# YyzHarry/imbalanced-regression

Hardware: NVIDIA H100
Metric: images/sec (higher is better)
Workload: dtype bf16

## Files before the change

imbalanced-regression_b200/_convlib.py:

```python
from ctypes import c_float, c_int, c_int64, c_size_t, c_void_p

import _lib

P = c_void_p
_I9 = [c_int] * 9

_lib.register({
    "dirb200_conv_prep_weights": (c_int, [P, c_int, c_int, c_int, c_int, c_int, P, P, P]),
    "dirb200_input_to_s2d": (c_int, [P, c_int, c_int, c_int, P, P]),
    "dirb200_conv_fprop": (c_int, [P, P, P] + _I9 + [c_int, P]),
    "dirb200_conv_dgrad": (c_int, [P, P, P] + _I9 + [P]),
    "dirb200_conv_wgrad_workspace_bytes": (c_size_t, _I9 + [c_int]),
    "dirb200_conv_wgrad": (c_int, [P, P, P, P, c_size_t] + _I9 + [c_int, c_int, P]),
    "dirb200_conv_plan": (c_int, _I9 + [c_int, c_int, P]),
    "dirb200_bn_eval_coeffs": (c_int, [c_int, P, P, c_float, P, P, P, P, P]),
    "dirb200_conv_fprop_bn_stats": (c_int, [P, P, P] + _I9 + [c_int, P, P, P]),
    "dirb200_conv_fprop_affine": (c_int, [P, P, P] + _I9 + [P, P, P, c_int, P]),
    "dirb200_conv_dgrad_bn_moments": (c_int, [P, P, P] + _I9 + [P, P, P, P, P, P]),
    "dirb200_bn_finalize_layout": (c_int, [P, P, c_int64, c_int, P, P, c_float, c_float, P, P, P, P, P, P, P]),
    "dirb200_bn_bwd_coeffs_layout": (c_int, [P, P, c_int64, c_int, P, P, P, P, P, P, P]),
})
```

imbalanced-regression_b200/csrc/conv.cuh:

```cuda
#pragma once
#include "common.cuh"

namespace dirb200 {

struct ConvShape {
  int n, h, w, cin, cout, kh, kw, stride, pad, ho, wo;
};

struct StatLayout {
  int rows, n_tiles, bn, group;
};

int conv_fprop(const __nv_bfloat16* x, const __nv_bfloat16* w, __nv_bfloat16* y, const ConvShape& s, bool stem,
               cudaStream_t st, float* stat_partial = nullptr, StatLayout* layout = nullptr);
struct ConvEpilogue {
  const float* scale;
  const float* shift;
  const __nv_bfloat16* residual;
  bool relu;
};
int conv_fprop_affine(const __nv_bfloat16* x, const __nv_bfloat16* w, __nv_bfloat16* out, const ConvShape& s,
                      const ConvEpilogue& epi, cudaStream_t st);
struct DgradBnMoments {
  const __nv_bfloat16* y;
  const float *scale, *shift;
  float* partial;
  StatLayout* layout;
};
bool conv_dgrad_fuses_bn_moments(const ConvShape& s);
int conv_dgrad(const __nv_bfloat16* dy, const __nv_bfloat16* wt, __nv_bfloat16* dx, const ConvShape& s,
               cudaStream_t st, const DgradBnMoments* bnm = nullptr);
int conv_wgrad_splits(const ConvShape& s);
size_t conv_wgrad_workspace_bytes(const ConvShape& s);
int conv_wgrad_partials(const __nv_bfloat16* x, const __nv_bfloat16* dy, float* partial, const ConvShape& s, bool stem,
                        int* splits_out, cudaStream_t st);
int wgrad_reduce(const float* workspace, int splits, float* dw, const ConvShape& s, bool stem, bool accumulate,
                 cudaStream_t st);
int conv_wgrad(const __nv_bfloat16* x, const __nv_bfloat16* dy, float* dw, float* workspace, const ConvShape& s,
               bool stem, bool accumulate, cudaStream_t st);
struct WgradReduceDesc {
  const float* partial;
  size_t w_off;
  int splits, cout, cin, kh, kw, stem;
};
int wgrad_reduce_all(const WgradReduceDesc* descs_dev, int nlayers, float* grads, cudaStream_t st);
struct PrepDesc {
  size_t w_off;
  int cout, cin, kh, kw, stem;
  __nv_bfloat16 *wf, *wd;
  FastDiv fd_cin, fd_cout, fd_taps;
};
inline PrepDesc make_prep_desc(size_t w_off, int cout, int cin, int kh, int kw, int stem, __nv_bfloat16* wf,
                               __nv_bfloat16* wd) {
  PrepDesc d{w_off, cout, cin, kh, kw, stem, wf, wd, {}, {}, {}};
  d.fd_cin = make_fastdiv((uint32_t)cin);
  d.fd_cout = make_fastdiv((uint32_t)cout);
  d.fd_taps = make_fastdiv((uint32_t)(kh * kw));
  return d;
}
int conv_plan(const ConvShape& s, bool stem, int op, int* plan);
int prep_weights_all(const float* params, const PrepDesc* descs_dev, int nlayers, cudaStream_t st);
int prep_weights(const float* w, int cout, int cin, int kh, int kw, bool stem, __nv_bfloat16* wf, __nv_bfloat16* wd,
                 cudaStream_t st);
int input_to_s2d(const float* x, int n, int h, int w, __nv_bfloat16* out, cudaStream_t st);

}
```

imbalanced-regression_b200/csrc/conv_api.cu:

```cuda
#include "common.cuh"
#include "conv.cuh"

namespace dirb200 {

__global__ void prep_weights_kernel(const float* __restrict__ w, int cout, int cin, int kh, int kw,
                                    __nv_bfloat16* __restrict__ wf, __nv_bfloat16* __restrict__ wd) {
  const int64_t total = (int64_t)cout * cin * kh * kw;
  for (int64_t i = blockIdx.x * (int64_t)blockDim.x + threadIdx.x; i < total; i += (int64_t)gridDim.x * blockDim.x) {
    int c = (int)(i % cin);
    int64_t t = i / cin;
    int s = (int)(t % kw); t /= kw;
    int r = (int)(t % kh);
    int co = (int)(t / kh);
    const float v = w[(((int64_t)co * cin + c) * kh + r) * kw + s];
    const __nv_bfloat16 b = __float2bfloat16_rn(v);
    wf[i] = b;
    if (wd) wd[(((int64_t)c * kh + r) * kw + s) * cout + co] = b;
  }
}

__global__ void prep_stem_weights_kernel(const float* __restrict__ w, int cout, __nv_bfloat16* __restrict__ wf) {
  const int total = cout * 256;
  for (int i = blockIdx.x * blockDim.x + threadIdx.x; i < total; i += gridDim.x * blockDim.x) {
    const int co = i >> 8, k = i & 255;
    const int rp = k >> 6, sp = (k >> 4) & 3, ph = (k >> 3) & 1, pw = (k >> 2) & 1, c = k & 3;
    const int r = 2 * rp + ph - 1, s = 2 * sp + pw - 1;
    float v = 0.f;
    if (c < 3 && r >= 0 && s >= 0 && r < 7 && s < 7) v = w[((co * 3 + c) * 7 + r) * 7 + s];
    wf[i] = __float2bfloat16_rn(v);
  }
}

__global__ void input_to_s2d_kernel(const float* __restrict__ x, int n, int h, int w, __nv_bfloat16* __restrict__ out) {
  const int h2 = h / 2, w2 = w / 2;
  const int64_t total = (int64_t)n * h2 * w2;
  for (int64_t i = blockIdx.x * (int64_t)blockDim.x + threadIdx.x; i < total; i += (int64_t)gridDim.x * blockDim.x) {
    const int xw = (int)(i % w2);
    const int yh = (int)((i / w2) % h2);
    const int b = (int)(i / ((int64_t)w2 * h2));
    __align__(16) __nv_bfloat16 v[16];
#pragma unroll
    for (int ph = 0; ph < 2; ++ph)
#pragma unroll
      for (int pw = 0; pw < 2; ++pw) {
#pragma unroll
        for (int c = 0; c < 3; ++c)
          v[(ph * 2 + pw) * 4 + c] =
              __float2bfloat16_rn(x[(((int64_t)b * 3 + c) * h + (2 * yh + ph)) * w + (2 * xw + pw)]);
        v[(ph * 2 + pw) * 4 + 3] = __float2bfloat16_rn(0.f);
      }
    uint4* o = reinterpret_cast<uint4*>(out + i * 16);
    o[0] = reinterpret_cast<uint4*>(v)[0];
    o[1] = reinterpret_cast<uint4*>(v)[1];
  }
}

__global__ void wgrad_reduce_kernel(const float* __restrict__ partial, int splits, int cout, int cin, int kh, int kw,
                                    int accumulate, float* __restrict__ dw) {
  const int64_t ktot = (int64_t)kh * kw * cin;
  const int64_t total = ktot * cout;
  const int64_t i = blockIdx.x * (int64_t)blockDim.x + threadIdx.x;
  if (i >= total) return;
  const int co = (int)(i / ktot);
  const int64_t k = i - (int64_t)co * ktot;
  float acc = 0.f;
  for (int sp = 0; sp < splits; ++sp) acc += partial[(int64_t)sp * total + i];
  const int c = (int)(k % cin);
  const int t = (int)(k / cin);
  float* o = dw + ((int64_t)co * cin + c) * (kh * kw) + t;
  *o = accumulate ? *o + acc : acc;
}

__global__ void wgrad_reduce_stem_kernel(const float* __restrict__ partial, int splits, int cout, int accumulate,
                                         float* __restrict__ dw) {
  const int total = 256 * cout;
  for (int i = blockIdx.x * blockDim.x + threadIdx.x; i < total; i += gridDim.x * blockDim.x) {
    const int co = i >> 8, k = i & 255;
    const int rp = k >> 6, sp_ = (k >> 4) & 3, ph = (k >> 3) & 1, pw = (k >> 2) & 1, c = k & 3;
    const int r = 2 * rp + ph - 1, s = 2 * sp_ + pw - 1;
    if (c >= 3 || r < 0 || s < 0) continue;
    float acc = 0.f;
    for (int sp = 0; sp < splits; ++sp) acc += partial[(int64_t)sp * total + i];
    float* o = dw + ((co * 3 + c) * 7 + r) * 7 + s;
    *o = accumulate ? *o + acc : acc;
  }
}

__global__ void __launch_bounds__(256)
wgrad_reduce_all_kernel(const WgradReduceDesc* __restrict__ descs, float* __restrict__ grads) {
  const WgradReduceDesc d = descs[blockIdx.y];
  float* dw = grads + d.w_off;
  if (d.stem) {
    const int total = 256 * d.cout;
    for (int i = blockIdx.x * blockDim.x + threadIdx.x; i < total; i += gridDim.x * blockDim.x) {
      const int co = i >> 8, k = i & 255;
      const int rp = k >> 6, sp_ = (k >> 4) & 3, ph = (k >> 3) & 1, pw = (k >> 2) & 1, c = k & 3;
      const int r = 2 * rp + ph - 1, s = 2 * sp_ + pw - 1;
      if (c >= 3 || r < 0 || s < 0) continue;
      float acc = 0.f;
      for (int sp = 0; sp < d.splits; ++sp) acc += d.partial[(int64_t)sp * total + i];
      dw[((co * 3 + c) * 7 + r) * 7 + s] += acc;
    }
    return;
  }
  const int64_t ktot = (int64_t)d.kh * d.kw * d.cin;
  const int64_t total = ktot * d.cout;
  const int taps = d.kh * d.kw;
  for (int64_t i = blockIdx.x * (int64_t)blockDim.x + threadIdx.x; i < total; i += (int64_t)gridDim.x * blockDim.x) {
    const float* p = d.partial + i;
    float a0 = 0.f, a1 = 0.f, a2 = 0.f, a3 = 0.f;
    int sp = 0;
    for (; sp + 4 <= d.splits; sp += 4) {
      a0 += p[(int64_t)sp * total];
      a1 += p[(int64_t)(sp + 1) * total];
      a2 += p[(int64_t)(sp + 2) * total];
      a3 += p[(int64_t)(sp + 3) * total];
    }
    for (; sp < d.splits; ++sp) a0 += p[(int64_t)sp * total];
    const int64_t co = i / ktot, k = i - co * ktot;
    const int c = (int)(k % d.cin), t = (int)(k / d.cin);
    dw[(co * d.cin + c) * taps + t] += (a0 + a1) + (a2 + a3);
  }
}

int wgrad_reduce_all(const WgradReduceDesc* descs_dev, int nlayers, float* grads, cudaStream_t st) {
  if (nlayers <= 0) return DIRB200_OK;
  wgrad_reduce_all_kernel<<<dim3(2 * num_sms(), nlayers), 256, 0, st>>>(descs_dev, grads);
  DIRB_LAUNCHED();
  return DIRB200_OK;
}

__global__ void prep_weights_all_kernel(const float* __restrict__ params, const PrepDesc* __restrict__ descs) {
  const PrepDesc d = descs[blockIdx.y];
  const float* w = params + d.w_off;
  if (d.stem) {
    const int total = d.cout * 256;
    for (int i = blockIdx.x * blockDim.x + threadIdx.x; i < total; i += gridDim.x * blockDim.x) {
      const int co = i >> 8, k = i & 255;
      const int rp = k >> 6, sp = (k >> 4) & 3, ph = (k >> 3) & 1, pw = (k >> 2) & 1, c = k & 3;
      const int r = 2 * rp + ph - 1, s = 2 * sp + pw - 1;
      float v = 0.f;
      if (c < 3 && r >= 0 && s >= 0 && r < 7 && s < 7) v = w[((co * 3 + c) * 7 + r) * 7 + s];
      d.wf[i] = __float2bfloat16_rn(v);
    }
    return;
  }
  const uint32_t taps = (uint32_t)(d.kh * d.kw);
  const uint32_t total = (uint32_t)d.cout * (uint32_t)d.cin * taps;
  const uint32_t stride = gridDim.x * blockDim.x;
  for (uint32_t i = blockIdx.x * blockDim.x + threadIdx.x; i < total; i += stride) {
    uint32_t t, c, co, tap;
    d.fd_cin.divmod(i, t, c);
    d.fd_taps.divmod(t, co, tap);
    d.wf[i] = __float2bfloat16_rn(w[((size_t)co * d.cin + c) * taps + tap]);
  }
  if (!d.wd) return;
  for (uint32_t i = blockIdx.x * blockDim.x + threadIdx.x; i < total; i += stride) {
    uint32_t t, c, co, tap;
    d.fd_cout.divmod(i, t, co);
    d.fd_taps.divmod(t, c, tap);
    d.wd[i] = __float2bfloat16_rn(w[((size_t)co * d.cin + c) * taps + tap]);
  }
}

int prep_weights_all(const float* params, const PrepDesc* descs_dev, int nlayers, cudaStream_t st) {
  prep_weights_all_kernel<<<dim3(96, nlayers), 256, 0, st>>>(params, descs_dev);
  DIRB_LAUNCHED();
  return DIRB200_OK;
}

static inline int grid1d(int64_t n, int block = 256) {
  int64_t g = (n + block - 1) / block;
  const int64_t cap = 8 * (int64_t)num_sms();
  return (int)(g < 1 ? 1 : (g > cap ? cap : g));
}

int prep_weights(const float* w, int cout, int cin, int kh, int kw, bool stem, __nv_bfloat16* wf, __nv_bfloat16* wd,
                 cudaStream_t st) {
  if (stem) {
    prep_stem_weights_kernel<<<grid1d((int64_t)cout * 256), 256, 0, st>>>(w, cout, wf);
  } else {
    prep_weights_kernel<<<grid1d((int64_t)cout * cin * kh * kw), 256, 0, st>>>(w, cout, cin, kh, kw, wf, wd);
  }
  DIRB_LAUNCHED();
  return DIRB200_OK;
}

int input_to_s2d(const float* x, int n, int h, int w, __nv_bfloat16* out, cudaStream_t st) {
  input_to_s2d_kernel<<<grid1d((int64_t)n * (h / 2) * (w / 2)), 256, 0, st>>>(x, n, h, w, out);
  DIRB_LAUNCHED();
  return DIRB200_OK;
}

int wgrad_reduce(const float* workspace, int splits, float* dw, const ConvShape& s, bool stem, bool accumulate,
                 cudaStream_t st) {
  if (stem)
    wgrad_reduce_stem_kernel<<<grid1d(256 * (int64_t)s.cout), 256, 0, st>>>(workspace, splits, s.cout, accumulate, dw);
  else
  {
    const int64_t total = (int64_t)s.kh * s.kw * s.cin * s.cout;
    wgrad_reduce_kernel<<<(unsigned)((total + 255) / 256), 256, 0, st>>>(workspace, splits, s.cout, s.cin, s.kh, s.kw,
                                                                         accumulate, dw);
  }
  DIRB_LAUNCHED();
  return DIRB200_OK;
}

int conv_wgrad(const __nv_bfloat16* x, const __nv_bfloat16* dy, float* dw, float* workspace, const ConvShape& s,
               bool stem, bool accumulate, cudaStream_t st) {
  int splits = 1;
  if (int rc = conv_wgrad_partials(x, dy, workspace, s, stem, &splits, st)) return rc;
  return wgrad_reduce(workspace, splits, dw, s, stem, accumulate, st);
}

static int to_shape(int n, int h, int w, int cin, int cout, int kh, int kw, int stride, int pad, int stem,
                    ConvShape* s) {
  if (stem) {
    DIRB_CHECK_ARG(cin == 3 && kh == 7 && kw == 7 && stride == 2 && pad == 3 && h % 2 == 0 && w % 2 == 0,
                   "stem conv must be 3->Cout 7x7 stride 2 pad 3 on even H, W");
    *s = ConvShape{n, h / 2, w / 2, 16, cout, 4, 4, 1, 2, h / 2, w / 2};
  } else {
    DIRB_CHECK_ARG(n > 0 && h > 0 && w > 0 && kh > 0 && kw > 0 && stride > 0 && pad >= 0, "bad conv shape");
    *s = ConvShape{n, h, w, cin, cout, kh, kw, stride, pad, (h + 2 * pad - kh) / stride + 1,
                   (w + 2 * pad - kw) / stride + 1};
  }
  return DIRB200_OK;
}

static int conv_job_shape_ok(const char* who, int k, int cout, int cin, int kh, int kw, int stem) {
  DIRB_CHECK_ARG(cout > 0 && cin > 0 && kh > 0 && kw > 0, "%s: job %d has a non-positive size (%d, %d, %d, %d)", who, k,
                 cout, cin, kh, kw);
  DIRB_CHECK_ARG(!stem || (cin == 3 && kh == 7 && kw == 7), "%s: job %d: the stem must be 3x7x7", who, k);
  const int64_t weights = (int64_t)cout * cin * kh * kw;
  DIRB_CHECK_ARG(weights < (int64_t(1) << 31) && (!stem || 256 * (int64_t)cout < (int64_t(1) << 31)),
                 "%s: job %d has 2^31 or more weights", who, k);
  return DIRB200_OK;
}

}

using namespace dirb200;

extern "C" {

int dirb200_conv_prep_weights(const float* w, int cout, int cin, int kh, int kw, int stem, void* w_fprop,
                              void* w_dgrad, void* stream) {
  DIRB_CHECK_ARG(w && w_fprop && cout > 0 && cin > 0, "conv_prep_weights: bad arguments");
  DIRB_CHECK_ARG(!stem || (cin == 3 && kh == 7 && kw == 7), "conv_prep_weights: stem must be 3x7x7");
  return prep_weights(w, cout, cin, kh, kw, stem != 0, (__nv_bfloat16*)w_fprop, (__nv_bfloat16*)w_dgrad,
                      as_stream(stream));
}

int dirb200_input_to_s2d(const float* x_nchw, int n, int h, int w, void* out_bf16, void* stream) {
  DIRB_CHECK_ARG(x_nchw && out_bf16 && n > 0 && h > 0 && w > 0 && h % 2 == 0 && w % 2 == 0,
                 "input_to_s2d: bad arguments");
  return input_to_s2d(x_nchw, n, h, w, (__nv_bfloat16*)out_bf16, as_stream(stream));
}

int dirb200_conv_fprop(const void* x, const void* w_fprop, void* y, int n, int h, int w, int cin, int cout, int kh,
                       int kw, int stride, int pad, int stem, void* stream) {
  DIRB_CHECK_ARG(x && w_fprop && y, "conv_fprop: null pointer");
  ConvShape s;
  if (int rc = to_shape(n, h, w, cin, cout, kh, kw, stride, pad, stem, &s)) return rc;
  return conv_fprop((const __nv_bfloat16*)x, (const __nv_bfloat16*)w_fprop, (__nv_bfloat16*)y, s, stem != 0,
                    as_stream(stream));
}

int dirb200_conv_dgrad(const void* dy, const void* w_dgrad, void* dx, int n, int h, int w, int cin, int cout, int kh,
                       int kw, int stride, int pad, void* stream) {
  DIRB_CHECK_ARG(dy && w_dgrad && dx, "conv_dgrad: null pointer");
  ConvShape s;
  if (int rc = to_shape(n, h, w, cin, cout, kh, kw, stride, pad, 0, &s)) return rc;
  return conv_dgrad((const __nv_bfloat16*)dy, (const __nv_bfloat16*)w_dgrad, (__nv_bfloat16*)dx, s,
                    as_stream(stream));
}

size_t dirb200_conv_wgrad_workspace_bytes(int n, int h, int w, int cin, int cout, int kh, int kw, int stride, int pad,
                                          int stem) {
  ConvShape s;
  if (to_shape(n, h, w, cin, cout, kh, kw, stride, pad, stem, &s)) return 0;
  return conv_wgrad_workspace_bytes(s);
}

int dirb200_conv_wgrad(const void* x, const void* dy, float* dw, void* workspace, size_t workspace_bytes, int n, int h,
                       int w, int cin, int cout, int kh, int kw, int stride, int pad, int stem, int accumulate,
                       void* stream) {
  DIRB_CHECK_ARG(x && dy && dw && workspace, "conv_wgrad: null pointer");
  ConvShape s;
  if (int rc = to_shape(n, h, w, cin, cout, kh, kw, stride, pad, stem, &s)) return rc;
  if (workspace_bytes < conv_wgrad_workspace_bytes(s)) {
    set_error("conv_wgrad: workspace too small (%zu < %zu)", workspace_bytes, conv_wgrad_workspace_bytes(s));
    return DIRB200_ERR_WORKSPACE;
  }
  return conv_wgrad((const __nv_bfloat16*)x, (const __nv_bfloat16*)dy, dw, (float*)workspace, s, stem != 0,
                    accumulate != 0, as_stream(stream));
}

static void layout_to_host(const StatLayout& l, int* layout_host) {
  layout_host[0] = l.rows; layout_host[1] = l.n_tiles; layout_host[2] = l.bn; layout_host[3] = l.group;
}

int dirb200_conv_fprop_bn_stats(const void* x, const void* w_fprop, void* y, int n, int h, int w, int cin, int cout,
                                int kh, int kw, int stride, int pad, int stem, float* partial, int* layout_host,
                                void* stream) {
  DIRB_CHECK_ARG(x && w_fprop && y && partial && layout_host, "conv_fprop_bn_stats: null pointer");
  ConvShape s;
  if (int rc = to_shape(n, h, w, cin, cout, kh, kw, stride, pad, stem, &s)) return rc;
  StatLayout lay{};
  if (int rc = conv_fprop((const __nv_bfloat16*)x, (const __nv_bfloat16*)w_fprop, (__nv_bfloat16*)y, s, stem != 0,
                          as_stream(stream), partial, &lay))
    return rc;
  layout_to_host(lay, layout_host);
  return DIRB200_OK;
}

int dirb200_conv_fprop_affine(const void* x, const void* w_fprop, void* out, int n, int h, int w, int cin, int cout,
                              int kh, int kw, int stride, int pad, const float* scale, const float* shift,
                              const void* residual, int relu, void* stream) {
  DIRB_CHECK_ARG(x && w_fprop && out, "conv_fprop_affine: null pointer");
  ConvShape s;
  if (int rc = to_shape(n, h, w, cin, cout, kh, kw, stride, pad, 0, &s)) return rc;
  return conv_fprop_affine((const __nv_bfloat16*)x, (const __nv_bfloat16*)w_fprop, (__nv_bfloat16*)out, s,
                           ConvEpilogue{scale, shift, (const __nv_bfloat16*)residual, relu != 0}, as_stream(stream));
}

int dirb200_conv_dgrad_bn_moments(const void* dy, const void* w_dgrad, void* dx, int n, int h, int w, int cin, int cout,
                                  int kh, int kw, int stride, int pad, const void* y_prev, const float* scale,
                                  const float* shift, float* partial, int* layout_host, void* stream) {
  DIRB_CHECK_ARG(dy && w_dgrad && dx && y_prev && scale && shift && partial && layout_host,
                 "conv_dgrad_bn_moments: null pointer");
  ConvShape s;
  if (int rc = to_shape(n, h, w, cin, cout, kh, kw, stride, pad, 0, &s)) return rc;
  StatLayout lay{};
  const DgradBnMoments bm{(const __nv_bfloat16*)y_prev, scale, shift, partial, &lay};
  if (int rc = conv_dgrad((const __nv_bfloat16*)dy, (const __nv_bfloat16*)w_dgrad, (__nv_bfloat16*)dx, s,
                          as_stream(stream), &bm))
    return rc;
  layout_to_host(lay, layout_host);
  return DIRB200_OK;
}

int dirb200_conv_plan(int n, int h, int w, int cin, int cout, int kh, int kw, int stride, int pad, int stem, int op,
                      int* plan7) {
  DIRB_CHECK_ARG(plan7 && op >= 0 && op <= 2, "conv_plan: bad arguments");
  ConvShape s;
  if (int rc = to_shape(n, h, w, cin, cout, kh, kw, stride, pad, stem, &s)) return rc;
  return conv_plan(s, stem != 0, op, plan7);
}

int dirb200_prep_weights_all(const float* params, const dirb200_prep_job* jobs_host, int njobs, void* stream) {
  DIRB_CHECK_ARG(params && jobs_host, "prep_weights_all: null pointer");
  DIRB_CHECK_ARG(njobs >= 1 && njobs <= 65535, "prep_weights_all: njobs must be 1 .. 65535 (got %d)", njobs);
  std::vector<PrepDesc> descs;
  for (int k = 0; k < njobs; ++k) {
    const dirb200_prep_job& j = jobs_host[k];
    DIRB_CHECK_ARG(j.w_fprop, "prep_weights_all: job %d has a null w_fprop", k);
    DIRB_CHECK_ARG(j.w_off >= 0, "prep_weights_all: job %d has a negative w_off", k);
    if (int rc = conv_job_shape_ok("prep_weights_all", k, j.cout, j.cin, j.kh, j.kw, j.stem)) return rc;
    DIRB_CHECK_ARG(!j.stem || !j.w_dgrad, "prep_weights_all: job %d: the stem has no dgrad operand (w_dgrad must be null)",
                   k);
    descs.push_back(make_prep_desc((size_t)j.w_off, j.cout, j.cin, j.kh, j.kw, j.stem ? 1 : 0,
                                   (__nv_bfloat16*)j.w_fprop, (__nv_bfloat16*)j.w_dgrad));
  }
  cudaStream_t st = as_stream(stream);
  return with_device_table(descs, st, [&](const PrepDesc* d) { return prep_weights_all(params, d, njobs, st); });
}

int dirb200_wgrad_reduce_all(const dirb200_wgrad_reduce_job* jobs_host, int njobs, float* grads, void* stream) {
  DIRB_CHECK_ARG(jobs_host && grads, "wgrad_reduce_all: null pointer");
  DIRB_CHECK_ARG(njobs >= 1 && njobs <= 65535, "wgrad_reduce_all: njobs must be 1 .. 65535 (got %d)", njobs);
  std::vector<WgradReduceDesc> descs;
  for (int k = 0; k < njobs; ++k) {
    const dirb200_wgrad_reduce_job& j = jobs_host[k];
    DIRB_CHECK_ARG(j.partial, "wgrad_reduce_all: job %d has a null partial", k);
    DIRB_CHECK_ARG(j.w_off >= 0, "wgrad_reduce_all: job %d has a negative w_off", k);
    DIRB_CHECK_ARG(j.splits >= 1, "wgrad_reduce_all: job %d: splits must be at least 1 (got %d)", k, j.splits);
    if (int rc = conv_job_shape_ok("wgrad_reduce_all", k, j.cout, j.cin, j.kh, j.kw, j.stem)) return rc;
    descs.push_back(WgradReduceDesc{j.partial, (size_t)j.w_off, j.splits, j.cout, j.cin, j.kh, j.kw, j.stem ? 1 : 0});
  }
  cudaStream_t st = as_stream(stream);
  return with_device_table(descs, st, [&](const WgradReduceDesc* d) { return wgrad_reduce_all(d, njobs, grads, st); });
}

}
```

imbalanced-regression_b200/csrc/conv_igemm.cu:

```cuda
#include <stdlib.h>
#include "common.cuh"
#include "tc.cuh"
#include "conv.cuh"

namespace dirb200 {
using namespace tc;

constexpr int BM = 128;
constexpr int BK = 64;
constexpr int kProducerThreads = 128;
constexpr int kThreads = 384;
constexpr int kMaxTaps = 25;
constexpr int kMaxSmemBytes = 232448;

struct IgemmParams {
  const __nv_bfloat16* src;
  int n, hs, ws, cs;
  int hm, wm;
  int kh, kw, stride, pad;
  int transposed;
  int cls_on, cls_py, cls_px, full_h, full_w;
  int ntaps_c;
  int tap_list[kMaxTaps];
  long long tap_eoff[kMaxTaps];
  unsigned short tap_r[kMaxTaps], tap_s[kMaxTaps];
  FastDiv fd_hw, fd_wm, fd_cpb, fd_kw, fd_ntiles, fd_persplit;
  int cpb;
  long long pixels;
  int num_kblocks;
  int kblocks_per_split;
  int total_chunks;
  int m_tiles, n_tiles;
  int num_tiles;
  int a_mode;
  int i2c_stride, i2c_lo;
  int ldc;
  void* out;
  float* stat_out;
  const float* epi_scale;
  const float* epi_shift;
  const __nv_bfloat16* epi_res;
  int epi_relu;
  const __nv_bfloat16* bst_y;
  const float* bst_scale;
  const float* bst_shift;
};

template <int BN, bool STAGED_EPI>
struct Cfg {
  static constexpr int kABytes = BM * BK * 2;
  static constexpr int kBBytes = BN * BK * 2;
  static constexpr int kStageBytes = kABytes + kBBytes;
  static constexpr int kStages = BN == 128 ? (STAGED_EPI ? 5 : 6) : 8;
  static constexpr int kBarOffset = kStages * kStageBytes;
  static constexpr int kStageRowBytes = BN * 2 + 16;
  static constexpr int kEpiWarpBytes = 16 * kStageRowBytes;
  static constexpr int kEpiOffset = kBarOffset + 256;
  static constexpr int kStatWarpBytes = 2 * BN * 4;
  static constexpr int kStatOffset = kEpiOffset + (STAGED_EPI ? 8 * kEpiWarpBytes : 0);
  static constexpr int kSmemBytes = kStatOffset + (STAGED_EPI ? 8 * kStatWarpBytes : 0) + 1024;
  static_assert(kSmemBytes <= kMaxSmemBytes, "shared memory budget");
};

__device__ __forceinline__ uint32_t pack_pixel(long long p, const IgemmParams& P) {
  if (p >= P.pixels) return 0u;
  uint32_t n, rem, y, x;
  P.fd_hw.divmod(static_cast<uint32_t>(p), n, rem);
  P.fd_wm.divmod(rem, y, x);
  return 0x80000000u | (n << 18) | (y << 9) | x;
}

struct RowPre {
  int nb, yb, xb;
};
__device__ __forceinline__ RowPre row_pre(const IgemmParams& P, uint32_t pk) {
  RowPre rp;
  const int n = (pk >> 18) & 0x1FFF;
  int y = (pk >> 9) & 0x1FF, x = pk & 0x1FF;
  if (P.cls_on) {
    y = 2 * y + P.cls_py;
    x = 2 * x + P.cls_px;
  }
  rp.nb = n * P.hs;
  if (!P.transposed) {
    rp.yb = y * P.stride - P.pad;
    rp.xb = x * P.stride - P.pad;
  } else {
    rp.yb = y + P.pad;
    rp.xb = x + P.pad;
  }
  if (!(pk >> 31)) rp.yb = -(1 << 28);
  return rp;
}

__device__ __forceinline__ const __nv_bfloat16* tap_source(const IgemmParams& P, const RowPre& rp, int r, int s,
                                                           int coff, bool& ok) {
  int hi, wi;
  ok = true;
  if (!P.transposed) {
    hi = rp.yb + r;
    wi = rp.xb + s;
  } else {
    hi = rp.yb - r;
    wi = rp.xb - s;
    if (P.stride == 2) {
      ok = ((hi | wi) & 1) == 0;
      hi >>= 1;
      wi >>= 1;
    }
  }
  ok = ok && static_cast<unsigned>(hi) < static_cast<unsigned>(P.hs) &&
       static_cast<unsigned>(wi) < static_cast<unsigned>(P.ws);
  return ok ? P.src + (static_cast<size_t>(rp.nb + hi) * P.ws + wi) * P.cs + coff : P.src;
}

template <int BN, bool WGRAD, bool STEM, bool ATMA = false, bool AFFINE = false, bool BSTAT = false>
__global__ void __launch_bounds__(kThreads, 1)
igemm_kernel(const __grid_constant__ CUtensorMap tmap_b, const __grid_constant__ CUtensorMap tmap_a,
             const IgemmParams P) {
  using C = Cfg<BN, !WGRAD>;
  static_assert(BN == 64 || BN == 128, "tile width: one m64n64 / m64n128 wgmma per warpgroup and k step");
  static_assert(!ATMA || !STEM, "TMA-fed A operand: not for the stem");
  static_assert(!AFFINE || (!WGRAD && !STEM), "folded-BN epilogue: non-stem fprop GEMMs only");
  static_assert(!BSTAT || (ATMA && !WGRAD && !AFFINE), "BN-backward moments in the epilogue: TMA-fed dgrad GEMMs only");
  extern __shared__ uint8_t smem_raw[];
  const uint32_t smem_base = (smem_u32(smem_raw) + 1023u) & ~1023u;
  uint8_t* const smem_gen = smem_raw + (smem_base - smem_u32(smem_raw));
  const uint32_t bar_base = smem_base + C::kBarOffset;
  auto a_addr = [&](int s) { return smem_base + s * C::kStageBytes; };
  auto b_addr = [&](int s) { return smem_base + s * C::kStageBytes + C::kABytes; };
  constexpr uint32_t nstages = C::kStages;
  auto full_bar = [&](int s) { return bar_base + 8u * s; };
  auto empty_bar = [&](int s) { return bar_base + 8u * (C::kStages + s); };
  const int warp = static_cast<int>(threadIdx.x >> 5), lane = threadIdx.x & 31;

  int tile_first, tile_end, tile_step, fixed_n = 0;
  if constexpr (WGRAD) {
    tile_first = blockIdx.x; tile_end = P.num_tiles; tile_step = gridDim.x;
  } else {
    uint32_t gi, nn;
    P.fd_ntiles.divmod(blockIdx.x, gi, nn);
    fixed_n = static_cast<int>(nn);
    tile_first = static_cast<int>(gi);
    tile_end = P.m_tiles;
    tile_step = static_cast<int>(P.fd_ntiles.div(gridDim.x - 1u - nn)) + 1;
  }
  auto decode_tile = [&](int t, int& split, int& m_tile, int& n_tile, int& kb_begin, int& nk) {
    if constexpr (WGRAD) {
      uint32_t sp, rem, mt, nt;
      P.fd_persplit.divmod(static_cast<uint32_t>(t), sp, rem);
      P.fd_ntiles.divmod(rem, mt, nt);
      split = static_cast<int>(sp);
      m_tile = static_cast<int>(mt);
      n_tile = static_cast<int>(nt);
      kb_begin = split * P.kblocks_per_split;
      const int kb_end = min(P.num_kblocks, kb_begin + P.kblocks_per_split);
      nk = max(0, kb_end - kb_begin);
    } else {
      split = 0;
      m_tile = t;
      n_tile = fixed_n;
      kb_begin = 0;
      nk = P.num_kblocks;
    }
  };

  if (threadIdx.x == 0) {
    for (int s = 0; s < C::kStages; ++s) {
      mbar_init(full_bar(s), ATMA ? 1 : kProducerThreads + 1);
      mbar_init(empty_bar(s), 8);
    }
    fence_barrier_init();
  }
  __syncthreads();

  if (warp < 4) {
    if constexpr (!ATMA) {
      const int j = lane & 7;
      const int q = lane >> 3;
      uint32_t rs = 0, rph = 0;
      for (int t = tile_first; t < tile_end; t += tile_step) {
        int split, m_tile, n_tile, kb_begin, nk;
        decode_tile(t, split, m_tile, n_tile, kb_begin, nk);
        const int n0 = n_tile * BN;
        long long off8[8];
        uint32_t mask8[8];
        int chunk_r = 0, chunk_s = 0, chunk_c0 = 0;
        bool chunk_ok = true;
        uint32_t tile_off = 0;
        if constexpr (!WGRAD) {
          const RowPre rp = row_pre(P, pack_pixel(static_cast<long long>(m_tile) * BM + warp * 32 + lane, P));
          const bool rvalid = rp.yb > -(1 << 27);
          int oy = rp.yb, ox = rp.xb;
          if (P.transposed && P.stride == 2) { oy >>= 1; ox >>= 1; }
          const long long my_off = (static_cast<long long>(rp.nb + oy) * P.ws + ox) * P.cs;
          uint32_t vy = 0, vx = 0;
          if (rvalid) {
            const int nky = P.kh, nkx = STEM ? 4 : P.kw;
            for (int r = 0; r < nky; ++r) {
              int h = P.transposed ? rp.yb - r : rp.yb + r;
              bool ok = true;
              if (P.transposed && P.stride == 2) { ok = (h & 1) == 0; h >>= 1; }
              vy |= (ok && static_cast<unsigned>(h) < static_cast<unsigned>(P.hs) ? 1u : 0u) << r;
            }
            for (int c = 0; c < nkx; ++c) {
              int w = P.transposed ? rp.xb - c : rp.xb + c;
              bool ok = true;
              if (P.transposed && P.stride == 2) { ok = (w & 1) == 0; w >>= 1; }
              vx |= (ok && static_cast<unsigned>(w) < static_cast<unsigned>(P.ws) ? 1u : 0u) << c;
            }
          }
          uint32_t my_mask;
          if constexpr (STEM) {
            my_mask = vy | (vx << 8);
          } else {
            my_mask = 0;
            for (int r = 0; r < P.kh; ++r)
              if ((vy >> r) & 1u) my_mask |= vx << (r * P.kw);
          }
#pragma unroll
          for (int i = 0; i < 8; ++i) {
            const int row = 4 * i + q;
            const long long o = __shfl_sync(0xffffffffu, my_off, row);
            const uint32_t m = __shfl_sync(0xffffffffu, my_mask, row);
            if constexpr (STEM) {
              off8[i] = o + (j >> 1) * P.cs + (j & 1) * 8;
              mask8[i] = ((m >> (8 + (j >> 1))) & 1u) ? (m & 0xFu) : 0u;
            } else {
              off8[i] = o + j * 8;
              mask8[i] = m;
            }
          }
          tile_off = warp * 32 * 128;
        } else {
          const int chunk = warp >> 1;
          const int gchunk = m_tile * 2 + chunk;
          chunk_ok = gchunk < P.total_chunks;
          if constexpr (STEM) {
            chunk_r = gchunk;
          } else {
            uint32_t tap, cb, cr, csx;
            P.fd_cpb.divmod(static_cast<uint32_t>(gchunk), tap, cb);
            P.fd_kw.divmod(tap, cr, csx);
            chunk_c0 = static_cast<int>(cb) * 64;
            chunk_r = static_cast<int>(cr);
            chunk_s = static_cast<int>(csx);
          }
          tile_off = chunk * 8192 + (warp & 1) * 32 * 128;
        }
        int tc = 0, cb = 0;
        long long stem_toff = 0;
        for (int it = 0; it < nk; ++it) {
          const int s = static_cast<int>(rs);
          mbar_wait(empty_bar(s), rph ^ 1u);
          if (++rs == nstages) { rs = 0; rph ^= 1u; }
          const int kb = kb_begin + it;
          const uint32_t dst_base = a_addr(s) + tile_off;
          int kcoord = kb;
          if constexpr (!WGRAD) {
            int tp;
            long long toff;
            if constexpr (STEM) {
              tp = kb;
              toff = stem_toff;
              stem_toff += static_cast<long long>(P.ws) * P.cs;
            } else {
              tp = P.tap_list[tc];
              toff = P.tap_eoff[tc] + cb * 64;
              kcoord = tp * P.cpb + cb;
              if (++cb == P.cpb) { cb = 0; ++tc; }
            }
#pragma unroll
            for (int i = 0; i < 8; ++i) {
              const int row = 4 * i + q;
              const bool ok = (mask8[i] >> tp) & 1u;
              const __nv_bfloat16* src = ok ? P.src + (off8[i] + toff) : P.src;
              cp_async16(dst_base + row * 128 + ((j ^ (row & 7)) << 4), src, ok ? 16u : 0u);
            }
          } else {
            const uint32_t mypk = chunk_ok ? pack_pixel(static_cast<long long>(kb) * 64 + (warp & 1) * 32 + lane, P) : 0u;
            const RowPre rp = row_pre(P, mypk);
            bool myok;
            const __nv_bfloat16* myptr = tap_source(P, rp, chunk_r, STEM ? 0 : chunk_s, STEM ? 0 : chunk_c0, myok);
            const unsigned long long myaddr = reinterpret_cast<unsigned long long>(myptr);
            uint32_t okbits;
            if constexpr (STEM) {
              okbits = 0;
              const bool rowok = (mypk >> 31) && static_cast<unsigned>(rp.yb + chunk_r) < static_cast<unsigned>(P.hs);
              for (int sp = 0; sp < 4; ++sp)
                okbits |= (rowok && static_cast<unsigned>(rp.xb + sp) < static_cast<unsigned>(P.ws) ? 1u : 0u) << sp;
            } else {
              okbits = myok ? 1u : 0u;
            }
            unsigned long long rowaddr = myaddr;
            if constexpr (STEM)
              rowaddr = reinterpret_cast<unsigned long long>(
                  P.src + ((static_cast<long long>(rp.nb + rp.yb + chunk_r) * P.ws + rp.xb) * P.cs));
#pragma unroll
            for (int i = 0; i < 8; ++i) {
              const int row = 4 * i + q;
              const unsigned long long a = __shfl_sync(0xffffffffu, rowaddr, row);
              const uint32_t okb = __shfl_sync(0xffffffffu, okbits, row);
              const bool ok = STEM ? ((okb >> (j >> 1)) & 1u) : (okb & 1u);
              const __nv_bfloat16* src = reinterpret_cast<const __nv_bfloat16*>(a) + j * 8;
              cp_async16(dst_base + row * 128 + ((j ^ (row & 7)) << 4), ok ? src : P.src, ok ? 16u : 0u);
            }
          }
          if (warp == 0) {
            if (elect_one()) {
              mbar_arrive_expect_tx(full_bar(s), C::kBBytes);
              if constexpr (!WGRAD) {
                tma_load_2d(b_addr(s), &tmap_b, full_bar(s), kcoord * BK, n0);
              } else {
#pragma unroll
                for (int i = 0; i < BN / 64; ++i)
                  tma_load_2d(b_addr(s) + i * 8192, &tmap_b, full_bar(s), n0 + 64 * i, kb * 64);
              }
            }
            __syncwarp();
          }
          cp_async_mbar_arrive_noinc(full_bar(s));
        }
      }
    } else if (warp == 0) {
      uint32_t rs = 0, rph = 0;
      for (int t = tile_first; t < tile_end; t += tile_step) {
        int split, m_tile, n_tile, kb_begin, nk;
        decode_tile(t, split, m_tile, n_tile, kb_begin, nk);
        const int n0 = n_tile * BN;
        int tile_w0 = 0, tile_h0 = 0, tile_n0 = 0;
        if constexpr (!WGRAD) {
          if (P.a_mode == 2) {
            uint32_t tn, rem, y0, x0;
            P.fd_hw.divmod(static_cast<uint32_t>(m_tile) * BM, tn, rem);
            P.fd_wm.divmod(rem, y0, x0);
            tile_n0 = static_cast<int>(tn);
            tile_w0 = static_cast<int>(x0) * P.i2c_stride + P.i2c_lo;
            tile_h0 = static_cast<int>(y0) * P.i2c_stride + P.i2c_lo;
          }
        }
        int tc = 0, cb = 0;
        for (int it = 0; it < nk; ++it) {
          const int s = static_cast<int>(rs);
          mbar_wait(empty_bar(s), rph ^ 1u);
          if (++rs == nstages) { rs = 0; rph ^= 1u; }
          const int kb = kb_begin + it;
          if (elect_one()) {
            if constexpr (!WGRAD) {
              mbar_arrive_expect_tx(full_bar(s), C::kBBytes + C::kABytes);
              if (P.a_mode == 1)
                tma_load_2d(a_addr(s), &tmap_a, full_bar(s), kb * BK, m_tile * BM);
              else
                tma_load_im2col_4d(a_addr(s), &tmap_a, full_bar(s), cb * BK, tile_w0, tile_h0, tile_n0,
                                   P.tap_s[tc], P.tap_r[tc]);
              tma_load_2d(b_addr(s), &tmap_b, full_bar(s), (P.tap_list[tc] * P.cpb + cb) * BK, n0);
            } else {
              const int nchunks = min(2, P.total_chunks - 2 * m_tile);
              mbar_arrive_expect_tx(full_bar(s), C::kBBytes + nchunks * 8192);
              if (P.a_mode == 1) {
                for (int i = 0; i < nchunks; ++i)
                  tma_load_2d(a_addr(s) + i * 8192, &tmap_a, full_bar(s), (2 * m_tile + i) * 64, kb * 64);
              } else {
                uint32_t n0i, rem, y0, x0;
                P.fd_hw.divmod(static_cast<uint32_t>(kb) * 64u, n0i, rem);
                P.fd_wm.divmod(rem, y0, x0);
                for (int i = 0; i < nchunks; ++i) {
                  uint32_t tap, cbk, r, sx;
                  P.fd_cpb.divmod(static_cast<uint32_t>(2 * m_tile + i), tap, cbk);
                  P.fd_kw.divmod(tap, r, sx);
                  tma_load_im2col_4d(a_addr(s) + i * 8192, &tmap_a, full_bar(s), static_cast<int>(cbk) * 64,
                                     static_cast<int>(x0) * P.i2c_stride + P.i2c_lo,
                                     static_cast<int>(y0) * P.i2c_stride + P.i2c_lo, static_cast<int>(n0i),
                                     static_cast<uint16_t>(sx), static_cast<uint16_t>(r));
                }
              }
#pragma unroll
              for (int i = 0; i < BN / 64; ++i)
                tma_load_2d(b_addr(s) + i * 8192, &tmap_b, full_bar(s), n0 + 64 * i, kb * 64);
            }
          }
          if constexpr (!WGRAD) {
            if (++cb == P.cpb) { cb = 0; ++tc; }
          }
          __syncwarp();
        }
      }
    }
    return;
  }

  const int g = (warp >> 2) - 1;
  const int wq = warp & 3;
  const int ew = g * 4 + wq;
  const int fr = lane >> 2, fc = 2 * (lane & 3);
  float* const stat_sm = reinterpret_cast<float*>(smem_gen + C::kStatOffset) + ew * (2 * BN);
  if constexpr (!WGRAD) {
    if (P.stat_out != nullptr)
      for (int i = lane; i < 2 * BN; i += 32) stat_sm[i] = 0.f;
  }
  constexpr uint32_t kLbo = WGRAD ? 8192u : 16u;
  constexpr uint32_t kadv = WGRAD ? (2048u >> 4) : (32u >> 4);
  constexpr int kT = WGRAD ? 1 : 0;
  float acc[BN / 2];
  uint32_t rs = 0, rph = 0;
  for (int t = tile_first; t < tile_end; t += tile_step) {
    int split, m_tile, n_tile, kb_begin, nk;
    decode_tile(t, split, m_tile, n_tile, kb_begin, nk);
    int prev = 0;
    for (int it = 0; it < nk; ++it) {
      const int s = static_cast<int>(rs);
      mbar_wait(full_bar(s), rph);
      if (++rs == nstages) { rs = 0; rph ^= 1u; }
      if constexpr (!ATMA) fence_proxy_async();
      const uint64_t adesc = make_smem_desc(a_addr(s) + g * 8192, kLbo, 1024u);
      const uint64_t bdesc = make_smem_desc(b_addr(s), kLbo, 1024u);
      wgmma_fence_operands(acc);
      wgmma_fence();
#pragma unroll
      for (int k = 0; k < BK / 16; ++k)
        wgmma_bf16<BN, kT, kT>(acc, adesc + static_cast<uint64_t>(k * kadv), bdesc + static_cast<uint64_t>(k * kadv),
                               (it > 0 || k > 0) ? 1u : 0u);
      wgmma_commit();
      wgmma_fence_operands(acc);
      if (it > 0) {
        wgmma_wait<1>();
        if (lane == 0) mbar_arrive(empty_bar(prev));
      }
      prev = s;
    }
    wgmma_wait<0>();
    wgmma_fence_operands(acc);
    if (nk > 0 && lane == 0) mbar_arrive(empty_bar(prev));
    const int n0 = n_tile * BN;

    if constexpr (!WGRAD) {
      const uint32_t stage_base = smem_base + C::kEpiOffset + ew * C::kEpiWarpBytes;
      const bool relu_now = AFFINE && P.epi_relu && P.epi_res == nullptr;
#pragma unroll
      for (int j = 0; j < BN / 8; ++j) {
        const int col = 8 * j + fc;
        float v0 = acc[4 * j], v1 = acc[4 * j + 1], v2 = acc[4 * j + 2], v3 = acc[4 * j + 3];
        if constexpr (AFFINE) {
          const float2 a = __ldg(reinterpret_cast<const float2*>(P.epi_scale + n0 + col));
          const float2 b = __ldg(reinterpret_cast<const float2*>(P.epi_shift + n0 + col));
          v0 = fmaf(v0, a.x, b.x); v1 = fmaf(v1, a.y, b.y); v2 = fmaf(v2, a.x, b.x); v3 = fmaf(v3, a.y, b.y);
          if (relu_now) { v0 = fmaxf(v0, 0.f); v1 = fmaxf(v1, 0.f); v2 = fmaxf(v2, 0.f); v3 = fmaxf(v3, 0.f); }
        }
        __nv_bfloat162 h0 = __floats2bfloat162_rn(v0, v1), h1 = __floats2bfloat162_rn(v2, v3);
        asm volatile("st.shared.b32 [%0], %1;" ::"r"(stage_base + fr * C::kStageRowBytes + col * 2),
                     "r"(*reinterpret_cast<uint32_t*>(&h0)) : "memory");
        asm volatile("st.shared.b32 [%0], %1;" ::"r"(stage_base + (fr + 8) * C::kStageRowBytes + col * 2),
                     "r"(*reinterpret_cast<uint32_t*>(&h1)) : "memory");
      }
      __syncwarp();
      constexpr int kLanesPerRow = BN * 2 / 16;
      constexpr int kRowsPerIter = 32 / kLanesPerRow;
      constexpr int kIters = 16 / kRowsPerIter;
      const int sub = lane / kLanesPerRow, col16 = lane % kLanesPerRow;
      const long long p0 = static_cast<long long>(m_tile) * BM + g * 64 + wq * 16;
      __nv_bfloat16* out_cols = reinterpret_cast<__nv_bfloat16*>(P.out) + n0 + col16 * 8;
#pragma unroll
      for (int i = 0; i < kIters; ++i) {
        const int rl = i * kRowsPerIter + sub;
        const long long p = p0 + rl;
        int orow = (p < P.pixels && nk > 0) ? static_cast<int>(p) : -1;
        if (orow >= 0 && P.cls_on) {
          const uint32_t pk = pack_pixel(p, P);
          const int n = (pk >> 18) & 0x1FFF, yy = (pk >> 9) & 0x1FF, xx = pk & 0x1FF;
          orow = (n * P.full_h + 2 * yy + P.cls_py) * P.full_w + 2 * xx + P.cls_px;
        }
        if (orow >= 0) {
          uint4 val;
          asm volatile("ld.shared.v4.b32 {%0, %1, %2, %3}, [%4];"
                       : "=r"(val.x), "=r"(val.y), "=r"(val.z), "=r"(val.w)
                       : "r"(stage_base + rl * C::kStageRowBytes + col16 * 16));
          if constexpr (AFFINE) {
            if (P.epi_res != nullptr) {
              const uint4 rv = *reinterpret_cast<const uint4*>(P.epi_res + n0 + col16 * 8 + static_cast<long long>(orow) * P.ldc);
              uint32_t o[4] = {val.x, val.y, val.z, val.w};
              const uint32_t rr[4] = {rv.x, rv.y, rv.z, rv.w};
#pragma unroll
              for (int e = 0; e < 4; ++e) {
                float lo = __uint_as_float(o[e] << 16) + __uint_as_float(rr[e] << 16);
                float hi = __uint_as_float(o[e] & 0xffff0000u) + __uint_as_float(rr[e] & 0xffff0000u);
                if (P.epi_relu) { lo = fmaxf(lo, 0.f); hi = fmaxf(hi, 0.f); }
                __nv_bfloat162 h = __floats2bfloat162_rn(lo, hi);
                o[e] = *reinterpret_cast<uint32_t*>(&h);
              }
              val = make_uint4(o[0], o[1], o[2], o[3]);
            }
          }
          *reinterpret_cast<uint4*>(out_cols + static_cast<long long>(orow) * P.ldc) = val;
        }
      }
      if (BSTAT || P.stat_out != nullptr) {
#pragma unroll
        for (int h = 0; h < BN / 64; ++h) {
          const int col = 2 * (lane + 32 * h);
          float s0 = 0.f, s1 = 0.f, q0 = 0.f, q1 = 0.f;
          float2 bsc = make_float2(0.f, 0.f), bsh = bsc;
          if constexpr (BSTAT) {
            bsc = __ldg(reinterpret_cast<const float2*>(P.bst_scale + n0 + col));
            bsh = __ldg(reinterpret_cast<const float2*>(P.bst_shift + n0 + col));
          }
#pragma unroll
          for (int r = 0; r < 16; ++r) {
            uint32_t w;
            asm volatile("ld.shared.b32 %0, [%1];" : "=r"(w) : "r"(stage_base + r * C::kStageRowBytes + col * 2));
            float g0 = __uint_as_float(w << 16), g1 = __uint_as_float(w & 0xffff0000u);
            if constexpr (BSTAT) {
              const long long p = p0 + r;
              const uint32_t yw = p < P.pixels ? __ldg(reinterpret_cast<const unsigned int*>(P.bst_y + p * P.ldc + n0 + col)) : 0u;
              const float y0 = __uint_as_float(yw << 16), y1 = __uint_as_float(yw & 0xffff0000u);
              if (!(fmaf(y0, bsc.x, bsh.x) > 0.f)) g0 = 0.f;
              if (!(fmaf(y1, bsc.y, bsh.y) > 0.f)) g1 = 0.f;
              s0 += g0; s1 += g1;
              q0 = fmaf(g0, y0, q0); q1 = fmaf(g1, y1, q1);
            } else {
              s0 += g0; s1 += g1;
              q0 = fmaf(g0, g0, q0); q1 = fmaf(g1, g1, q1);
            }
          }
          stat_sm[col] += s0;
          stat_sm[col + 1] += s1;
          stat_sm[BN + col] += q0;
          stat_sm[BN + col + 1] += q1;
        }
      }
      __syncwarp();
    } else {
      const int ktot = P.total_chunks * 64;
      const int krow = m_tile * BM + g * 64 + wq * 16 + fr;
      float* out = reinterpret_cast<float*>(P.out) + (static_cast<size_t>(split) * P.ldc + n0) * ktot;
#pragma unroll
      for (int j = 0; j < BN / 8; ++j) {
        const size_t c0 = static_cast<size_t>(8 * j + fc) * ktot;
#pragma unroll
        for (int e = 0; e < 2; ++e) {
          if (krow < ktot) out[c0 + e * ktot + krow] = nk > 0 ? acc[4 * j + e] : 0.f;
          if (krow + 8 < ktot) out[c0 + e * ktot + krow + 8] = nk > 0 ? acc[4 * j + 2 + e] : 0.f;
        }
      }
    }
  }
  if constexpr (!WGRAD) {
    if (P.stat_out != nullptr) {
      asm volatile("bar.sync 1, 256;" ::: "memory");
      const float* all = reinterpret_cast<const float*>(smem_gen + C::kStatOffset);
      float* dst = P.stat_out + static_cast<size_t>(blockIdx.x) * 2 * P.ldc + fixed_n * BN;
      for (int o = static_cast<int>(threadIdx.x) - kProducerThreads; o < 2 * BN; o += kThreads - kProducerThreads) {
        const int k = o / BN, col = o - k * BN;
        const float v = ((all[o] + all[2 * BN + o]) + (all[4 * BN + o] + all[6 * BN + o])) +
                        ((all[8 * BN + o] + all[10 * BN + o]) + (all[12 * BN + o] + all[14 * BN + o]));
        dst[static_cast<size_t>(k) * P.ldc + col] = v;
      }
    }
  }
}

typedef CUresult (*EncodeTiledFn)(CUtensorMap*, CUtensorMapDataType, cuuint32_t, void*, const cuuint64_t*,
                                  const cuuint64_t*, const cuuint32_t*, const cuuint32_t*, CUtensorMapInterleave,
                                  CUtensorMapSwizzle, CUtensorMapL2promotion, CUtensorMapFloatOOBfill);

static EncodeTiledFn encode_fn() {
  static EncodeTiledFn fn = nullptr;
  if (!fn) {
    void* p = nullptr;
    cudaDriverEntryPointQueryResult q;
    if (cudaGetDriverEntryPoint("cuTensorMapEncodeTiled", &p, cudaEnableDefault, &q) == cudaSuccess &&
        q == cudaDriverEntryPointSuccess)
      fn = reinterpret_cast<EncodeTiledFn>(p);
  }
  return fn;
}

int make_tmap_bf16_2d(CUtensorMap* tm, const void* ptr, uint64_t inner, uint64_t outer, uint64_t row_stride_bytes,
                      uint32_t box_outer) {
  EncodeTiledFn fn = encode_fn();
  if (!fn) {
    set_error("cuTensorMapEncodeTiled entry point not available");
    return DIRB200_ERR_CUDA;
  }
  cuuint64_t dims[2] = {inner, outer};
  cuuint64_t strides[1] = {row_stride_bytes};
  cuuint32_t box[2] = {64, box_outer};
  cuuint32_t estr[2] = {1, 1};
  CUresult r = fn(tm, CU_TENSOR_MAP_DATA_TYPE_BFLOAT16, 2, const_cast<void*>(ptr), dims, strides, box, estr,
                  CU_TENSOR_MAP_INTERLEAVE_NONE, CU_TENSOR_MAP_SWIZZLE_128B, CU_TENSOR_MAP_L2_PROMOTION_L2_256B,
                  CU_TENSOR_MAP_FLOAT_OOB_FILL_NONE);
  if (r != CUDA_SUCCESS) {
    set_error("cuTensorMapEncodeTiled failed (%d) inner=%llu outer=%llu stride=%llu", (int)r,
              (unsigned long long)inner, (unsigned long long)outer, (unsigned long long)row_stride_bytes);
    return DIRB200_ERR_CUDA;
  }
  return DIRB200_OK;
}

typedef CUresult (*EncodeIm2colFn)(CUtensorMap*, CUtensorMapDataType, cuuint32_t, void*, const cuuint64_t*,
                                   const cuuint64_t*, const int*, const int*, cuuint32_t, cuuint32_t, const cuuint32_t*,
                                   CUtensorMapInterleave, CUtensorMapSwizzle, CUtensorMapL2promotion,
                                   CUtensorMapFloatOOBfill);
int make_tmap_im2col_bf16(CUtensorMap* tm, const void* ptr, int c, int w, int h, int n, int lower_w, int lower_h,
                          int upper_w, int upper_h, int trav, int pixels_per_col) {
  static EncodeIm2colFn fn = nullptr;
  if (!fn) {
    void* p = nullptr;
    cudaDriverEntryPointQueryResult q;
    if (cudaGetDriverEntryPoint("cuTensorMapEncodeIm2col", &p, cudaEnableDefault, &q) == cudaSuccess &&
        q == cudaDriverEntryPointSuccess)
      fn = reinterpret_cast<EncodeIm2colFn>(p);
  }
  if (!fn) {
    set_error("cuTensorMapEncodeIm2col entry point not available");
    return DIRB200_ERR_CUDA;
  }
  cuuint64_t dims[4] = {(cuuint64_t)c, (cuuint64_t)w, (cuuint64_t)h, (cuuint64_t)n};
  cuuint64_t strides[3] = {(cuuint64_t)c * 2, (cuuint64_t)w * c * 2, (cuuint64_t)h * w * c * 2};
  int lower[2] = {lower_w, lower_h}, upper[2] = {upper_w, upper_h};
  cuuint32_t estr[4] = {1, (cuuint32_t)trav, (cuuint32_t)trav, 1};
  CUresult r = fn(tm, CU_TENSOR_MAP_DATA_TYPE_BFLOAT16, 4, const_cast<void*>(ptr), dims, strides, lower, upper, 64,
                  (cuuint32_t)pixels_per_col, estr, CU_TENSOR_MAP_INTERLEAVE_NONE, CU_TENSOR_MAP_SWIZZLE_128B,
                  CU_TENSOR_MAP_L2_PROMOTION_L2_256B, CU_TENSOR_MAP_FLOAT_OOB_FILL_NONE);
  if (r != CUDA_SUCCESS) {
    set_error("cuTensorMapEncodeIm2col failed (%d) c=%d w=%d h=%d n=%d lower=%d,%d upper=%d,%d stride=%d", (int)r, c, w, h,
              n, lower_w, lower_h, upper_w, upper_h, trav);
    return DIRB200_ERR_CUDA;
  }
  int drv = 0;
  if (cudaDriverGetVersion(&drv) == cudaSuccess && drv <= 13010 && (size_t)c * w * h * n * 2 < 131072)
    reinterpret_cast<uint64_t*>(tm)[1] &= ~(1ull << 21);
  return DIRB200_OK;
}
static thread_local StatLayout t_last_layout{};

static IgemmParams finish_params(const IgemmParams& P) {
  IgemmParams Q = P;
  Q.fd_hw = make_fastdiv(static_cast<uint32_t>(Q.hm * Q.wm));
  Q.fd_wm = make_fastdiv(static_cast<uint32_t>(Q.wm));
  Q.fd_cpb = make_fastdiv(static_cast<uint32_t>(Q.cpb > 0 ? Q.cpb : 1));
  Q.fd_kw = make_fastdiv(static_cast<uint32_t>(Q.kw > 0 ? Q.kw : 1));
  Q.fd_ntiles = make_fastdiv(static_cast<uint32_t>(Q.n_tiles > 0 ? Q.n_tiles : 1));
  Q.fd_persplit = make_fastdiv(static_cast<uint32_t>(Q.m_tiles * Q.n_tiles > 0 ? Q.m_tiles * Q.n_tiles : 1));
  const int nt = Q.ntaps_c < kMaxTaps ? Q.ntaps_c : kMaxTaps;
  for (int i = 0; i < kMaxTaps; ++i) {
    Q.tap_eoff[i] = 0;
    Q.tap_r[i] = Q.tap_s[i] = 0;
  }
  for (int i = 0; i < nt && Q.kw > 0; ++i) {
    const int tp = Q.tap_list[i];
    int r = tp / Q.kw, sx = tp - r * Q.kw;
    if (Q.transposed && Q.cls_on) {
      Q.tap_r[i] = static_cast<unsigned short>((Q.cls_py + Q.pad - r) / 2 - Q.i2c_lo);
      Q.tap_s[i] = static_cast<unsigned short>((Q.cls_px + Q.pad - sx) / 2 - Q.i2c_lo);
      r >>= 1; sx >>= 1;
      Q.tap_eoff[i] = -static_cast<long long>(r * Q.ws + sx) * Q.cs;
    } else if (Q.transposed) {
      Q.tap_r[i] = static_cast<unsigned short>(Q.kh - 1 - r);
      Q.tap_s[i] = static_cast<unsigned short>(Q.kw - 1 - sx);
      if (Q.stride == 2) { r >>= 1; sx >>= 1; }
      Q.tap_eoff[i] = -static_cast<long long>(r * Q.ws + sx) * Q.cs;
    } else {
      Q.tap_r[i] = static_cast<unsigned short>(r);
      Q.tap_s[i] = static_cast<unsigned short>(sx);
      Q.tap_eoff[i] = static_cast<long long>(r * Q.ws + sx) * Q.cs;
    }
  }
  return Q;
}

template <int BN, bool WGRAD, bool STEM, bool ATMA = false, bool AFFINE = false, bool BSTAT = false>
static int launch_igemm_impl(const CUtensorMap& tm, const CUtensorMap& tma, const IgemmParams& Qin, cudaStream_t st) {
  using C = Cfg<BN, !WGRAD>;
  const IgemmParams Q = finish_params(Qin);
  static bool configured = false;
  if (!configured) {
    DIRB_CUDA(cudaFuncSetAttribute(igemm_kernel<BN, WGRAD, STEM, ATMA, AFFINE, BSTAT>,
                                   cudaFuncAttributeMaxDynamicSharedMemorySize, C::kSmemBytes));
    configured = true;
  }
  int grid = Q.num_tiles < num_sms() ? Q.num_tiles : num_sms();
  if (!WGRAD && grid < Q.n_tiles) grid = Q.n_tiles;
  t_last_layout = StatLayout{grid, Q.n_tiles, BN, 1};
  igemm_kernel<BN, WGRAD, STEM, ATMA, AFFINE, BSTAT><<<grid, kThreads, C::kSmemBytes, st>>>(tm, tma, Q);
  DIRB_LAUNCHED();
  return DIRB200_OK;
}

template <int BN, bool WGRAD, bool STEM>
static int launch_igemm(const CUtensorMap& tm, const IgemmParams& P, int m_tiles, int splits, cudaStream_t st,
                        const CUtensorMap* tma = nullptr) {
  IgemmParams Q = P;
  Q.m_tiles = m_tiles;
  Q.num_tiles = m_tiles * P.n_tiles * splits;
  if constexpr (!STEM) {
    if (tma) {
      if constexpr (!WGRAD) {
        if (Q.epi_scale != nullptr) return launch_igemm_impl<BN, false, false, true, true>(tm, *tma, Q, st);
        if (Q.bst_y != nullptr) return launch_igemm_impl<BN, false, false, true, false, true>(tm, *tma, Q, st);
      }
      return launch_igemm_impl<BN, WGRAD, false, true>(tm, *tma, Q, st);
    }
  }
  if constexpr (!WGRAD && !STEM) {
    if (Q.epi_scale != nullptr) return launch_igemm_impl<BN, false, false, false, true>(tm, tm, Q, st);
  }
  if (Q.epi_scale != nullptr || Q.bst_y != nullptr) {
    set_error("conv: the BN-backward moments epilogue needs a TMA-fed A operand; the folded-BN one a non-stem fprop");
    return DIRB200_ERR_ARG;
  }
  return launch_igemm_impl<BN, WGRAD, STEM>(tm, tm, Q, st);
}

static int pick_bn(int n_dim) { return n_dim % 128 == 0 ? 128 : 64; }

#define DISPATCH_BN(bn, WG, ST, ...) \
  ((bn) == 128 ? launch_igemm<128, WG, ST>(__VA_ARGS__) : launch_igemm<64, WG, ST>(__VA_ARGS__))

static int check_shape(const ConvShape& s, bool stem, const char* who) {
  DIRB_CHECK_ARG(s.n > 0 && s.h > 0 && s.w > 0 && s.kh > 0 && s.kw > 0 && s.stride > 0 && s.pad >= 0,
                 "%s: bad conv shape", who);
  DIRB_CHECK_ARG(s.cout % 64 == 0, "%s: Cout must be a multiple of 64 (got %d)", who, s.cout);
  DIRB_CHECK_ARG(static_cast<long long>(s.n) * s.h * s.w < (1LL << 31) && static_cast<long long>(s.n) * s.ho * s.wo < (1LL << 31),
                 "%s: more than 2^31 pixels", who);
  if (stem)
    DIRB_CHECK_ARG(s.cin == 16 && s.kh == 4 && s.kw == 4 && s.stride == 1, "%s: stem expects the 4x4x16 s2d form", who);
  else
    DIRB_CHECK_ARG(s.cin % 64 == 0, "%s: Cin must be a multiple of 64 (got %d)", who, s.cin);
  return DIRB200_OK;
}

static bool atma_enabled() {
  static const bool on = [] {
    const char* e = getenv("DIRB200_ATMA");
    return !(e != nullptr && e[0] == '0');
  }();
  return on;
}
static bool is_plain_gemm(const ConvShape& s, bool stem) {
  return !stem && s.kh == 1 && s.kw == 1 && s.stride == 1 && s.pad == 0 && atma_enabled();
}
static bool im2col_enabled() {
  static const bool on = [] {
    const char* e = getenv("DIRB200_IM2COL");
    return !(e != nullptr && e[0] == '0');
  }();
  return on && atma_enabled();
}

static int conv_fprop_impl(const __nv_bfloat16* x, const __nv_bfloat16* w, __nv_bfloat16* y, const ConvShape& s, bool stem,
                           cudaStream_t st, float* stat_partial, const ConvEpilogue* epi);

int conv_fprop(const __nv_bfloat16* x, const __nv_bfloat16* w, __nv_bfloat16* y, const ConvShape& s, bool stem,
               cudaStream_t st, float* stat_partial, StatLayout* layout) {
  const int rc = conv_fprop_impl(x, w, y, s, stem, st, stat_partial, nullptr);
  if (layout) *layout = t_last_layout;
  return rc;
}

int conv_fprop_affine(const __nv_bfloat16* x, const __nv_bfloat16* w, __nv_bfloat16* out, const ConvShape& s,
                      const ConvEpilogue& epi, cudaStream_t st) {
  DIRB_CHECK_ARG(epi.scale && epi.shift, "conv_fprop_affine: scale / shift missing");
  return conv_fprop_impl(x, w, out, s, false, st, nullptr, &epi);
}

static int conv_fprop_impl(const __nv_bfloat16* x, const __nv_bfloat16* w, __nv_bfloat16* y, const ConvShape& s, bool stem,
                           cudaStream_t st, float* stat_partial, const ConvEpilogue* epi) {
  if (int rc = check_shape(s, stem, "conv_fprop")) return rc;
  const int ktot = s.kh * s.kw * s.cin;
  IgemmParams P{};
  P.src = x; P.n = s.n; P.hs = s.h; P.ws = s.w; P.cs = s.cin; P.hm = s.ho; P.wm = s.wo;
  P.kh = s.kh; P.kw = s.kw; P.stride = s.stride; P.pad = s.pad; P.transposed = 0;
  P.cpb = stem ? 1 : s.cin / 64;
  P.pixels = static_cast<long long>(s.n) * s.ho * s.wo;
  P.num_kblocks = ktot / 64;
  P.ntaps_c = s.kh * s.kw;
  DIRB_CHECK_ARG(stem || P.ntaps_c <= kMaxTaps, "conv_fprop: at most %d filter taps (got %dx%d)", kMaxTaps, s.kh, s.kw);
  for (int i = 0; i < kMaxTaps; ++i) P.tap_list[i] = i;
  P.ldc = s.cout; P.out = y;
  P.stat_out = stat_partial;
  if (epi) {
    P.epi_scale = epi->scale; P.epi_shift = epi->shift; P.epi_res = epi->residual; P.epi_relu = epi->relu ? 1 : 0;
  }
  const int m_tiles = static_cast<int>((P.pixels + BM - 1) / BM);
  const int bn = pick_bn(s.cout);
  P.n_tiles = s.cout / bn;
  CUtensorMap tm, ta;
  bool tma_fed = false;
  if (is_plain_gemm(s, stem)) {
    if (int rc = make_tmap_bf16_2d(&ta, x, s.cin, static_cast<uint64_t>(P.pixels), static_cast<uint64_t>(s.cin) * 2, BM))
      return rc;
    P.a_mode = 1;
    tma_fed = true;
  } else if (!stem && im2col_enabled()) {
    if (int rc = make_tmap_im2col_bf16(&ta, x, s.cin, s.w, s.h, s.n, -s.pad, -s.pad, s.pad - (s.kw - 1),
                                       s.pad - (s.kh - 1), s.stride, BM))
      return rc;
    P.a_mode = 2; P.i2c_stride = s.stride; P.i2c_lo = -s.pad;
    tma_fed = true;
  }
  if (int rc = make_tmap_bf16_2d(&tm, w, ktot, s.cout, static_cast<uint64_t>(ktot) * 2, bn)) return rc;
  if (stem) return DISPATCH_BN(bn, false, true, tm, P, m_tiles, 1, st);
  if (tma_fed) return DISPATCH_BN(bn, false, false, tm, P, m_tiles, 1, st, &ta);
  return DISPATCH_BN(bn, false, false, tm, P, m_tiles, 1, st);
}

bool conv_dgrad_fuses_bn_moments(const ConvShape& s) {
  return s.stride == 1 && (is_plain_gemm(s, false) || (im2col_enabled() && s.kh == s.kw));
}

int conv_dgrad(const __nv_bfloat16* dy, const __nv_bfloat16* wt, __nv_bfloat16* dx, const ConvShape& s,
               cudaStream_t st, const DgradBnMoments* bnm) {
  if (int rc = check_shape(s, false, "conv_dgrad")) return rc;
  DIRB_CHECK_ARG(!bnm || (conv_dgrad_fuses_bn_moments(s) && bnm->y && bnm->scale && bnm->shift && bnm->partial),
                 "conv_dgrad: BN-backward moments are fused into TMA-fed stride-1 dgrads only");
  DIRB_CHECK_ARG(s.stride == 1 || s.stride == 2, "conv_dgrad: stride must be 1 or 2 (got %d)", s.stride);
  DIRB_CHECK_ARG(s.kh * s.kw <= (s.stride == 1 ? kMaxTaps : 9), "conv_dgrad: at most %d filter taps (stride 2: 9; got %dx%d)",
                 kMaxTaps, s.kh, s.kw);
  const int ktot = s.kh * s.kw * s.cout;
  IgemmParams P{};
  P.src = dy; P.n = s.n; P.hs = s.ho; P.ws = s.wo; P.cs = s.cout; P.hm = s.h; P.wm = s.w;
  P.kh = s.kh; P.kw = s.kw; P.stride = s.stride; P.pad = s.pad; P.transposed = 1;
  P.cpb = s.cout / 64;
  P.ldc = s.cin; P.out = dx;
  if (bnm) {
    P.bst_y = bnm->y; P.bst_scale = bnm->scale; P.bst_shift = bnm->shift; P.stat_out = bnm->partial;
  }
  const int bn = pick_bn(s.cin);
  CUtensorMap tm;
  if (int rc = make_tmap_bf16_2d(&tm, wt, ktot, s.cin, static_cast<uint64_t>(ktot) * 2, bn)) return rc;
  if (s.stride == 1) {
    P.pixels = static_cast<long long>(s.n) * s.h * s.w;
    P.ntaps_c = s.kh * s.kw;
    for (int i = 0; i < kMaxTaps; ++i) P.tap_list[i] = i;
    P.num_kblocks = ktot / 64;
    const int m_tiles = static_cast<int>((P.pixels + BM - 1) / BM);
    P.n_tiles = s.cin / bn;
    CUtensorMap ta;
    bool tma_fed = false;
    if (is_plain_gemm(s, false)) {
      if (int rc = make_tmap_bf16_2d(&ta, dy, s.cout, static_cast<uint64_t>(P.pixels), static_cast<uint64_t>(s.cout) * 2, BM))
        return rc;
      P.a_mode = 1;
      tma_fed = true;
    } else if (im2col_enabled() && s.kh == s.kw) {
      const int lo = s.pad - (s.kh - 1);
      if (int rc = make_tmap_im2col_bf16(&ta, dy, s.cout, s.wo, s.ho, s.n, lo, lo, lo + s.w - s.wo, lo + s.h - s.ho, 1, BM))
        return rc;
      P.a_mode = 2; P.i2c_stride = 1; P.i2c_lo = lo;
      tma_fed = true;
    }
    const int rc = tma_fed ? DISPATCH_BN(bn, false, false, tm, P, m_tiles, 1, st, &ta)
                           : DISPATCH_BN(bn, false, false, tm, P, m_tiles, 1, st);
    if (bnm && bnm->layout) *bnm->layout = t_last_layout;
    return rc;
  }
  bool need_zero = false;
  for (int cls = 0; cls < 4; ++cls) {
    const int py = cls >> 1, px = cls & 1;
    int nt = 0;
    for (int r = 0; r < s.kh; ++r)
      for (int q = 0; q < s.kw; ++q)
        if (((py + s.pad - r) & 1) == 0 && ((px + s.pad - q) & 1) == 0) ++nt;
    if (nt == 0) need_zero = true;
  }
  if (need_zero)
    DIRB_CUDA(cudaMemsetAsync(dx, 0, static_cast<size_t>(s.n) * s.h * s.w * s.cin * sizeof(__nv_bfloat16), st));
  for (int cls = 0; cls < 4; ++cls) {
    IgemmParams Q = P;
    Q.cls_on = 1; Q.cls_py = cls >> 1; Q.cls_px = cls & 1; Q.full_h = s.h; Q.full_w = s.w;
    Q.hm = (s.h - Q.cls_py + 1) / 2;
    Q.wm = (s.w - Q.cls_px + 1) / 2;
    Q.ntaps_c = 0;
    for (int r = 0; r < s.kh; ++r)
      for (int q = 0; q < s.kw; ++q)
        if (((Q.cls_py + s.pad - r) & 1) == 0 && ((Q.cls_px + s.pad - q) & 1) == 0) Q.tap_list[Q.ntaps_c++] = r * s.kw + q;
    if (Q.ntaps_c == 0 || Q.hm <= 0 || Q.wm <= 0) continue;
    Q.pixels = static_cast<long long>(s.n) * Q.hm * Q.wm;
    Q.num_kblocks = Q.ntaps_c * Q.cpb;
    const int m_tiles = static_cast<int>((Q.pixels + BM - 1) / BM);
    Q.n_tiles = s.cin / bn;
    if (im2col_enabled()) {
      int lo = 1 << 20;
      for (int i = 0; i < Q.ntaps_c; ++i) {
        const int r = Q.tap_list[i] / s.kw, q = Q.tap_list[i] % s.kw;
        const int orr = (Q.cls_py + s.pad - r) / 2, oq = (Q.cls_px + s.pad - q) / 2;
        lo = orr < lo ? orr : lo;
        lo = oq < lo ? oq : lo;
      }
      CUtensorMap ta;
      if (int rc = make_tmap_im2col_bf16(&ta, dy, s.cout, s.wo, s.ho, s.n, lo, lo, lo + Q.wm - s.wo, lo + Q.hm - s.ho, 1, BM))
        return rc;
      Q.a_mode = 2; Q.i2c_stride = 1; Q.i2c_lo = lo;
      if (int rc = DISPATCH_BN(bn, false, false, tm, Q, m_tiles, 1, st, &ta)) return rc;
      continue;
    }
    if (int rc = DISPATCH_BN(bn, false, false, tm, Q, m_tiles, 1, st)) return rc;
  }
  return DIRB200_OK;
}

static int wgrad_bn(const ConvShape& s) { return pick_bn(s.cout); }

int conv_wgrad_splits(const ConvShape& s) {
  const long long pixels = static_cast<long long>(s.n) * s.ho * s.wo;
  const int kblocks = static_cast<int>((pixels + 63) / 64);
  const int chunks = s.kh * s.kw * s.cin / 64;
  const int bn = wgrad_bn(s);
  const int m_tiles = (chunks + 1) / 2;
  const int tiles = m_tiles * (s.cout / bn);
  const int sms = num_sms();
  int max_splits = (kblocks + 7) / 8;
  if (max_splits < 1) max_splits = 1;
  int hi = (4 * sms + tiles - 1) / tiles;
  if (hi > max_splits) hi = max_splits;
  int best = 1;
  long long best_cost = -1;
  for (int sp = 1; sp <= hi; ++sp) {
    const long long waves = (static_cast<long long>(tiles) * sp + sms - 1) / sms;
    const long long per = (kblocks + sp - 1) / sp;
    const long long cost = waves * (per + 6);
    if (best_cost < 0 || cost < best_cost) {
      best_cost = cost;
      best = sp;
    }
  }
  return best;
}

size_t conv_wgrad_workspace_bytes(const ConvShape& s) {
  return static_cast<size_t>(conv_wgrad_splits(s)) * s.kh * s.kw * s.cin * s.cout * sizeof(float);
}

int conv_wgrad_partials(const __nv_bfloat16* x, const __nv_bfloat16* dy, float* partial, const ConvShape& s, bool stem,
                        int* splits_out, cudaStream_t st) {
  if (int rc = check_shape(s, stem, "conv_wgrad")) return rc;
  IgemmParams P{};
  P.src = x; P.n = s.n; P.hs = s.h; P.ws = s.w; P.cs = s.cin; P.hm = s.ho; P.wm = s.wo;
  P.kh = s.kh; P.kw = s.kw; P.stride = s.stride; P.pad = s.pad; P.transposed = 0;
  P.cpb = stem ? 1 : s.cin / 64;
  P.pixels = static_cast<long long>(s.n) * s.ho * s.wo;
  P.num_kblocks = static_cast<int>((P.pixels + 63) / 64);
  P.total_chunks = s.kh * s.kw * s.cin / 64;
  P.ntaps_c = s.kh * s.kw;
  DIRB_CHECK_ARG(stem || P.ntaps_c <= kMaxTaps, "conv_wgrad: at most %d filter taps (got %dx%d)", kMaxTaps, s.kh, s.kw);
  for (int i = 0; i < kMaxTaps; ++i) P.tap_list[i] = i;
  const int splits = conv_wgrad_splits(s);
  P.kblocks_per_split = (P.num_kblocks + splits - 1) / splits;
  P.ldc = s.cout; P.out = partial;
  const int bn = wgrad_bn(s);
  P.n_tiles = s.cout / bn;
  const int m_tiles = (P.total_chunks + 1) / 2;
  *splits_out = splits;
  CUtensorMap tm;
  if (int rc = make_tmap_bf16_2d(&tm, dy, s.cout, static_cast<uint64_t>(P.pixels), static_cast<uint64_t>(s.cout) * 2, 64))
    return rc;
  if (stem) return DISPATCH_BN(bn, true, true, tm, P, m_tiles, splits, st);
  if (is_plain_gemm(s, stem)) {
    CUtensorMap ta;
    if (int rc = make_tmap_bf16_2d(&ta, x, s.cin, static_cast<uint64_t>(P.pixels), static_cast<uint64_t>(s.cin) * 2, 64))
      return rc;
    P.a_mode = 1;
    return DISPATCH_BN(bn, true, false, tm, P, m_tiles, splits, st, &ta);
  }
  if (im2col_enabled()) {
    CUtensorMap ta;
    if (int rc = make_tmap_im2col_bf16(&ta, x, s.cin, s.w, s.h, s.n, -s.pad, -s.pad, s.pad - (s.kw - 1),
                                       s.pad - (s.kh - 1), s.stride, 64))
      return rc;
    P.a_mode = 2; P.i2c_stride = s.stride; P.i2c_lo = -s.pad;
    return DISPATCH_BN(bn, true, false, tm, P, m_tiles, splits, st, &ta);
  }
  return DISPATCH_BN(bn, true, false, tm, P, m_tiles, splits, st);
}

int conv_plan(const ConvShape& s, bool stem, int op, int* plan) {
  for (int i = 0; i < 7; ++i) plan[i] = 0;
  plan[4] = plan[5] = 1;
  if (int rc = check_shape(s, stem, "conv_plan")) return rc;
  if (op == 2) {
    plan[0] = wgrad_bn(s);
    plan[4] = conv_wgrad_splits(s);
    plan[2] = stem ? 0 : (is_plain_gemm(s, stem) ? 1 : (im2col_enabled() ? 2 : 0));
    return DIRB200_OK;
  }
  const bool dgrad = op == 1;
  DIRB_CHECK_ARG(!(dgrad && stem), "conv_plan: the stem has no data gradient");
  const int n_dim = dgrad ? s.cin : s.cout;
  plan[0] = pick_bn(n_dim);
  if (dgrad && s.stride == 2) {
    int launches = 0;
    for (int cls = 0; cls < 4; ++cls) {
      const int py = cls >> 1, px = cls & 1;
      int nt = 0;
      for (int r = 0; r < s.kh; ++r)
        for (int q = 0; q < s.kw; ++q)
          if (((py + s.pad - r) & 1) == 0 && ((px + s.pad - q) & 1) == 0) ++nt;
      const int hm = (s.h - py + 1) / 2, wm = (s.w - px + 1) / 2;
      if (nt == 0 || hm <= 0 || wm <= 0) continue;
      ++launches;
    }
    plan[2] = im2col_enabled() ? 2 : 0; plan[5] = launches;
    return DIRB200_OK;
  }
  const bool tma_fed = is_plain_gemm(s, stem) || (!stem && im2col_enabled() && (!dgrad || s.kh == s.kw));
  plan[2] = stem ? 0 : (is_plain_gemm(s, stem) ? 1 : (tma_fed ? 2 : 0));
  plan[6] = dgrad && conv_dgrad_fuses_bn_moments(s);
  return DIRB200_OK;
}

}
```

imbalanced-regression_b200/csrc/tc.cuh:

```cuda
#pragma once
#include <cuda.h>
#include <stdint.h>

namespace dirb200 {
namespace tc {

__device__ __forceinline__ uint32_t smem_u32(const void* p) {
  return static_cast<uint32_t>(__cvta_generic_to_shared(p));
}

__device__ __forceinline__ void mbar_init(uint32_t bar, uint32_t count) {
  asm volatile("mbarrier.init.shared::cta.b64 [%0], %1;" ::"r"(bar), "r"(count) : "memory");
}
__device__ __forceinline__ void fence_barrier_init() {
  asm volatile("fence.mbarrier_init.release.cluster;" ::: "memory");
}
__device__ __forceinline__ void mbar_arrive(uint32_t bar) {
  asm volatile("mbarrier.arrive.shared::cta.b64 _, [%0];" ::"r"(bar) : "memory");
}
__device__ __forceinline__ void mbar_arrive_expect_tx(uint32_t bar, uint32_t bytes) {
  asm volatile("mbarrier.arrive.expect_tx.shared::cta.b64 _, [%0], %1;" ::"r"(bar), "r"(bytes) : "memory");
}
__device__ __forceinline__ bool mbar_try_wait(uint32_t bar, uint32_t parity) {
  uint32_t ok;
  asm volatile(
      "{\n"
      ".reg .pred p;\n"
      "mbarrier.try_wait.parity.shared::cta.b64 p, [%1], %2;\n"
      "selp.u32 %0, 1, 0, p;\n"
      "}\n"
      : "=r"(ok)
      : "r"(bar), "r"(parity)
      : "memory");
  return ok != 0;
}
__device__ __forceinline__ void mbar_wait(uint32_t bar, uint32_t parity) {
  if (mbar_try_wait(bar, parity)) return;
  unsigned long long t0;
  asm volatile("mov.u64 %0, %%globaltimer;" : "=l"(t0));
  while (!mbar_try_wait(bar, parity)) {
    unsigned long long t1;
    asm volatile("mov.u64 %0, %%globaltimer;" : "=l"(t1));
    if (t1 - t0 > 4000000000ull) __trap();
  }
}

__device__ __forceinline__ bool elect_one() {
  uint32_t pred;
  asm volatile(
      "{\n"
      ".reg .pred P;\n"
      "elect.sync _|P, 0xffffffff;\n"
      "selp.u32 %0, 1, 0, P;\n"
      "}\n"
      : "=r"(pred));
  return pred != 0;
}

__device__ __forceinline__ void cp_async16(uint32_t dst, const void* src, uint32_t src_bytes) {
  asm volatile("cp.async.cg.shared.global [%0], [%1], 16, %2;" ::"r"(dst), "l"(src), "r"(src_bytes) : "memory");
}
__device__ __forceinline__ void cp_async_mbar_arrive_noinc(uint32_t bar) {
  asm volatile("cp.async.mbarrier.arrive.noinc.shared::cta.b64 [%0];" ::"r"(bar) : "memory");
}
__device__ __forceinline__ void fence_proxy_async() { asm volatile("fence.proxy.async.shared::cta;" ::: "memory"); }

__device__ __forceinline__ void tma_load_2d(uint32_t dst, const CUtensorMap* tmap, uint32_t bar, int c0, int c1) {
  asm volatile(
      "cp.async.bulk.tensor.2d.shared::cluster.global.mbarrier::complete_tx::bytes [%0], [%1, {%3, %4}], [%2];"
      ::"r"(dst), "l"(tmap), "r"(bar), "r"(c0), "r"(c1)
      : "memory");
}

__device__ __forceinline__ void tma_load_im2col_4d(uint32_t dst, const CUtensorMap* tmap, uint32_t bar, int c, int w,
                                                   int h, int n, uint16_t off_w, uint16_t off_h) {
  asm volatile(
      "cp.async.bulk.tensor.4d.shared::cluster.global.im2col.mbarrier::complete_tx::bytes"
      " [%0], [%1, {%3, %4, %5, %6}], [%2], {%7, %8};"
      ::"r"(dst), "l"(tmap), "r"(bar), "r"(c), "r"(w), "r"(h), "r"(n), "h"(off_w), "h"(off_h)
      : "memory");
}

__device__ __forceinline__ void wgmma_fence() { asm volatile("wgmma.fence.sync.aligned;" ::: "memory"); }
__device__ __forceinline__ void wgmma_commit() { asm volatile("wgmma.commit_group.sync.aligned;" ::: "memory"); }
template <int N>
__device__ __forceinline__ void wgmma_wait() {
  asm volatile("wgmma.wait_group.sync.aligned %0;" ::"n"(N) : "memory");
}
template <int R>
__device__ __forceinline__ void wgmma_fence_operands(float (&d)[R]) {
#pragma unroll
  for (int i = 0; i < R; ++i) asm volatile("" : "+f"(d[i])::"memory");
}

#define DIRB_F4(i) "+f"(d[i]), "+f"(d[i + 1]), "+f"(d[i + 2]), "+f"(d[i + 3])
#define DIRB_F16(i) DIRB_F4(i), DIRB_F4(i + 4), DIRB_F4(i + 8), DIRB_F4(i + 12)
#define DIRB_R8(a, b, c, e, f, g, h, k) "%" #a ", %" #b ", %" #c ", %" #e ", %" #f ", %" #g ", %" #h ", %" #k ", "
template <int TA, int TB>
__device__ __forceinline__ void wgmma_m64n64(float (&d)[32], uint64_t adesc, uint64_t bdesc, uint32_t accumulate) {
  asm volatile(
      "{\n.reg .pred p;\nsetp.ne.b32 p, %34, 0;\n"
      "wgmma.mma_async.sync.aligned.m64n64k16.f32.bf16.bf16 {"
      DIRB_R8(0, 1, 2, 3, 4, 5, 6, 7) DIRB_R8(8, 9, 10, 11, 12, 13, 14, 15) DIRB_R8(16, 17, 18, 19, 20, 21, 22, 23)
      "%24, %25, %26, %27, %28, %29, %30, %31}, %32, %33, p, 1, 1, %35, %36;\n}\n"
      : DIRB_F16(0), DIRB_F16(16)
      : "l"(adesc), "l"(bdesc), "r"(accumulate), "n"(TA), "n"(TB));
}
template <int TA, int TB>
__device__ __forceinline__ void wgmma_m64n128(float (&d)[64], uint64_t adesc, uint64_t bdesc, uint32_t accumulate) {
  asm volatile(
      "{\n.reg .pred p;\nsetp.ne.b32 p, %66, 0;\n"
      "wgmma.mma_async.sync.aligned.m64n128k16.f32.bf16.bf16 {"
      DIRB_R8(0, 1, 2, 3, 4, 5, 6, 7) DIRB_R8(8, 9, 10, 11, 12, 13, 14, 15) DIRB_R8(16, 17, 18, 19, 20, 21, 22, 23)
      DIRB_R8(24, 25, 26, 27, 28, 29, 30, 31) DIRB_R8(32, 33, 34, 35, 36, 37, 38, 39) DIRB_R8(40, 41, 42, 43, 44, 45, 46, 47)
      DIRB_R8(48, 49, 50, 51, 52, 53, 54, 55)
      "%56, %57, %58, %59, %60, %61, %62, %63}, %64, %65, p, 1, 1, %67, %68;\n}\n"
      : DIRB_F16(0), DIRB_F16(16), DIRB_F16(32), DIRB_F16(48)
      : "l"(adesc), "l"(bdesc), "r"(accumulate), "n"(TA), "n"(TB));
}
#undef DIRB_R8
#undef DIRB_F16
#undef DIRB_F4
template <int BN, int TA, int TB>
__device__ __forceinline__ void wgmma_bf16(float (&d)[BN / 2], uint64_t adesc, uint64_t bdesc, uint32_t accumulate) {
  if constexpr (BN == 128) wgmma_m64n128<TA, TB>(d, adesc, bdesc, accumulate);
  else wgmma_m64n64<TA, TB>(d, adesc, bdesc, accumulate);
}

__device__ __forceinline__ uint64_t make_smem_desc(uint32_t saddr, uint32_t lbo_bytes, uint32_t sbo_bytes) {
  uint64_t d = 0;
  d |= static_cast<uint64_t>((saddr & 0x3FFFFu) >> 4);
  d |= static_cast<uint64_t>((lbo_bytes >> 4) & 0x3FFFu) << 16;
  d |= static_cast<uint64_t>((sbo_bytes >> 4) & 0x3FFFu) << 32;
  d |= static_cast<uint64_t>(1) << 62;
  return d;
}

}
}
```

include/dirb200.h:

```cpp
#ifndef DIRB200_H
#define DIRB200_H

#include <stddef.h>
#include <stdint.h>

#ifdef __cplusplus
extern "C" {
#endif

#define DIRB200_OK 0
#define DIRB200_ERR_ARG (-1)
#define DIRB200_ERR_CUDA (-2)
#define DIRB200_ERR_WORKSPACE (-3)

#define DIRB200_BIN_AGE 0
#define DIRB200_BIN_DEPTH10 1
#define DIRB200_BIN_EDGES5 2

#define DIRB200_LOSS_MSE 0
#define DIRB200_LOSS_L1 1
#define DIRB200_LOSS_FOCAL_MSE 2
#define DIRB200_LOSS_FOCAL_L1 3
#define DIRB200_LOSS_HUBER 4
#define DIRB200_ACT_SIGMOID 0
#define DIRB200_ACT_TANH 1

#define DIRB200_REWEIGHT_SQRT_INV 1
#define DIRB200_REWEIGHT_INVERSE 2

const char* dirb200_last_error(void);
int dirb200_version(void);
int64_t dirb200_launch_count(void);


int dirb200_fds_label_flags(const float* labels, int64_t n, int bucket_num, int bucket_start,
                            int bin_rule, int32_t* flags, void* stream);

int dirb200_fds_bin_rows(const float* labels, int64_t n, int bucket_num, int bucket_start,
                         int bin_rule, const int32_t* flags, int32_t* bins_out, void* stream);

size_t dirb200_fds_accumulate_workspace_bytes(int64_t n, int nb);

int dirb200_fds_accumulate(const float* features, const int32_t* bins, int64_t n, int d, int nb,
                           double* sums, double* sumsq, int64_t* counts,
                           void* workspace, size_t workspace_bytes, void* stream);

int dirb200_fds_set_profiling(int enabled);
int dirb200_fds_last_accumulate_kernel_ms(float* ms_out);

int dirb200_fds_finalize(const double* sums, const double* sumsq, const int64_t* counts, int nb, int d,
                         float* running_mean, float* running_var, float* num_samples_tracked,
                         double momentum, int first_update, void* stream);

int dirb200_fds_smooth_tables(const float* src, int nb, int d, const float* window_host, int ks,
                              float* dst, void* stream);

int dirb200_fds_calibrate_fwd(float* x, const float* labels, int64_t b, int d, int bucket_num,
                              int bucket_start, int bin_rule, const float* m1, const float* v1,
                              const float* m2, const float* v2, float clip_min, float clip_max,
                              int32_t* rowbin_out, int32_t* flags_scratch ,
                              void* stream);

int dirb200_fds_fill_empty(const int64_t* counts, int nb, int d, float* running_mean, float* running_var,
                           void* stream);

int dirb200_fds_calibrate_bwd(int bin_rule, const float* grad_out, const int32_t* rowbin, int64_t b, int d,
                              const float* v1, const float* v2, float clip_min, float clip_max,
                              float* grad_in, void* stream);


size_t dirb200_loss_workspace_bytes(int64_t n);

int dirb200_loss_fwd_bwd(int kind, const float* pred, const float* target, const float* weight, int64_t n,
                         float beta, float gamma, int activate, float grad_scale,
                         float* loss_out, float* grad_out, void* workspace, size_t workspace_bytes,
                         void* stream);


int dirb200_lds_histogram(const float* labels, int64_t n, int max_target, int64_t* hist, void* stream);

int dirb200_lds_weights(const float* labels, int64_t n, int max_target, int reweight,
                        const double* window_host, int ks, const int64_t* hist,
                        double* scratch, float* weights_out, void* stream);

int dirb200_lds_weights_sharded(const float* labels, int64_t n, int64_t n_total, int max_target, int reweight,
                                const double* window_host, int ks, const int64_t* hist, double* scratch,
                                float* weights_out, void* stream);

int dirb200_lds_table_lookup(const float* values, int64_t n, float mult, int max_bin, const float* table,
                             float* weights_out, void* stream);

size_t dirb200_bn_workspace_bytes(int c);
int dirb200_bn_train_fwd(const void* y, int64_t rows, int c, const float* gamma, const float* beta, float eps,
                         float momentum, float* running_mean, float* running_var, int relu, void* out, float* save_mean,
                         float* save_invstd, float* scale_shift, void* workspace, void* stream);
int dirb200_bn_eval_coeffs(int c, const float* gamma, const float* beta, float eps, const float* running_mean,
                           const float* running_var, float* scale, float* shift, void* stream);
int dirb200_bn_train_bwd(const void* grad_out, const void* y, int64_t rows, int c, const float* gamma,
                         const float* save_mean, const float* save_invstd, const float* scale_shift, int relu,
                         float* grad_gamma, float* grad_beta, void* grad_y, void* workspace, void* stream);
int dirb200_maxpool3x3s2_fwd(const void* x, int n, int h, int w, int c, void* out, uint8_t* argmax, void* stream);
int dirb200_maxpool3x3s2_bwd(const void* grad_out, const uint8_t* argmax, int n, int h, int w, int c, void* grad_x,
                             void* stream);
int dirb200_avgpool_fwd(const void* x, int n, int hw, int c, float* out, void* stream);
int dirb200_avgpool_bwd(const float* grad_out, int n, int hw, int c, void* grad_x, void* stream);

int dirb200_upsample_bilinear_fwd(const void* x, int n, int h, int w, int c, int ho, int wo, void* out, void* stream);
int dirb200_upsample_bilinear_bwd(const void* dy, int n, int h, int w, int c, int ho, int wo, void* dx, void* stream);
int dirb200_copy_channels(const void* src, int src_stride, int src_off, void* dst, int dst_stride, int dst_off, int c,
                          int64_t pixels, void* stream);
int dirb200_depth_head_fwd(const void* x, const float* w, const float* b, float* y, int n, int h, int wd, int c,
                           void* stream);
int dirb200_depth_head_dgrad(const float* dy, const float* w, void* dx, int n, int h, int wd, int c, void* stream);
size_t dirb200_depth_head_wgrad_workspace_bytes(int n, int h, int wd, int c);
int dirb200_depth_head_wgrad(const void* x, const float* dy, float* dw, float* db, void* workspace,
                             size_t workspace_bytes, int n, int h, int wd, int c, void* stream);

int dirb200_augment_batch(const uint8_t* images, const int* crop_yx, const uint8_t* flip, int n, int size, int pad,
                          float mean, float stdv, float* out, void* stream);

size_t dirb200_depth_augment_workspace_bytes(int n, int h, int w, int crop_h, int crop_w);
int dirb200_depth_augment_batch(const uint8_t* images, const void* depths, int depth_u16, int n, int h, int w,
                                int crop_h, int crop_w, int depth_h, int depth_w, const uint8_t* flip,
                                const double* affine, const float* rgb_offset, const int* jitter_order,
                                const float* jitter_alpha, const float* mean_std, const float* bucket_weights,
                                int n_buckets, float* image_out, float* depth_out, float* weight_out,
                                uint8_t* debug_crop, float* debug_mean, void* workspace, size_t workspace_bytes,
                                void* stream);

int dirb200_int_label_histogram(const float* labels, int64_t n, int nbins, int64_t* hist, void* stream);

int dirb200_shot_metrics(const float* preds, const float* labels, int64_t n, const int64_t* train_hist, int nbins,
                         int many_shot_thr, int low_shot_thr, double* out16, void* stream);

size_t dirb200_depth_metrics_workspace_bytes(int64_t n_images, int h, int w);
int dirb200_depth_metrics_accumulate(const float* pred, int ph, int pw, const float* target, const uint8_t* mask,
                                     int64_t n_images, int h, int w, const uint8_t* group_of_bin, int nbins,
                                     double* acc, void* workspace, size_t workspace_bytes, void* stream);

size_t dirb200_stsb_shot_metrics_workspace_bytes(int64_t n);
int dirb200_stsb_shot_metrics(const float* preds, const float* labels, int64_t n, void* workspace,
                              size_t workspace_bytes, double* out24, void* stream);


int dirb200_conv_prep_weights(const float* w, int cout, int cin, int kh, int kw, int stem,
                              void* w_fprop, void* w_dgrad, void* stream);

int dirb200_input_to_s2d(const float* x_nchw, int n, int h, int w, void* out_bf16, void* stream);

int dirb200_conv_fprop(const void* x, const void* w_fprop, void* y, int n, int h, int w, int cin,
                       int cout, int kh, int kw, int stride, int pad, int stem, void* stream);

int dirb200_conv_dgrad(const void* dy, const void* w_dgrad, void* dx, int n, int h, int w, int cin,
                       int cout, int kh, int kw, int stride, int pad, void* stream);

int dirb200_conv_plan(int n, int h, int w, int cin, int cout, int kh, int kw, int stride, int pad, int stem, int op,
                      int* plan7);
size_t dirb200_conv_wgrad_workspace_bytes(int n, int h, int w, int cin, int cout, int kh, int kw,
                                          int stride, int pad, int stem);

int dirb200_conv_wgrad(const void* x, const void* dy, float* dw, void* workspace, size_t workspace_bytes,
                       int n, int h, int w, int cin, int cout, int kh, int kw, int stride, int pad,
                       int stem, int accumulate, void* stream);


int dirb200_conv_fprop_bn_stats(const void* x, const void* w_fprop, void* y, int n, int h, int w, int cin, int cout,
                                int kh, int kw, int stride, int pad, int stem, float* partial, int* layout_host,
                                void* stream);
int dirb200_conv_fprop_affine(const void* x, const void* w_fprop, void* out, int n, int h, int w, int cin, int cout,
                              int kh, int kw, int stride, int pad, const float* scale, const float* shift,
                              const void* residual, int relu, void* stream);
int dirb200_conv_dgrad_bn_moments(const void* dy, const void* w_dgrad, void* dx, int n, int h, int w, int cin, int cout,
                                  int kh, int kw, int stride, int pad, const void* y_prev, const float* scale,
                                  const float* shift, float* partial, int* layout_host, void* stream);
int dirb200_bn_finalize_layout(const float* partial, const int* layout_host, int64_t rows, int c, const float* gamma,
                               const float* beta, float eps, float momentum, float* running_mean, float* running_var,
                               float* mean_out, float* invstd_out, float* scale_out, float* shift_out, void* stream);
int dirb200_bn_bwd_coeffs_layout(const float* partial, const int* layout_host, int64_t rows, int c, const float* mean,
                                 const float* invstd, const float* gamma, float* grad_gamma, float* grad_beta,
                                 float* coef_out, void* stream);


int dirb200_layer_bn_stats(const void* y, int64_t rows, int c, float* partial, int* nblocks_host, void* stream);
int dirb200_layer_bn_apply(const void* y, const float* scale, const float* shift, const void* res, const void* res_y,
                           const float* res_scale, const float* res_shift, int relu, int64_t rows, int c, void* out,
                           uint8_t* mask_out, void* stream);
int dirb200_layer_bn_bwd_reduce(const void* g1, const void* g2, const void* g3, const void* y, const void* y2,
                                const float* scale, const float* shift, const uint8_t* mask, int64_t rows, int c,
                                int g2_h, int g2_w, void* dz_out, float* partial, int* nblocks_host, void* stream);
int dirb200_layer_bn_bwd_coeffs(const float* partial, int nblocks, int k, int gslot, int64_t rows, int c,
                                const float* mean, const float* invstd, const float* gamma, float* grad_gamma,
                                float* grad_beta, float* coef_out, void* stream);
int dirb200_layer_bn_bwd_apply(const void* g1, const void* g2, const void* y, const float* coef, const void* y2,
                               const float* coef2, const float* scale, const float* shift, const uint8_t* mask,
                               int64_t rows, int c, int g2_h, int g2_w, void* dy, void* dy2, void* dz_out,
                               void* stream);
int dirb200_layer_bn_relu_maxpool_fwd(const void* y, const float* scale, const float* shift, int n, int h, int w, int c,
                                      void* out, uint8_t* argmax, void* stream);
int dirb200_layer_maxpool_bwd(const void* g1, const void* g2, const uint8_t* argmax, int n, int h, int w, int c,
                              void* dx, void* stream);


typedef struct dirb200_prep_job {
  int64_t w_off;
  int cout, cin, kh, kw, stem;
  void* w_fprop;
  void* w_dgrad;
} dirb200_prep_job;
int dirb200_prep_weights_all(const float* params, const dirb200_prep_job* jobs_host, int njobs, void* stream);

typedef struct dirb200_wgrad_reduce_job {
  const float* partial;
  int64_t w_off;
  int splits, cout, cin, kh, kw, stem;
} dirb200_wgrad_reduce_job;
int dirb200_wgrad_reduce_all(const dirb200_wgrad_reduce_job* jobs_host, int njobs, float* grads, void* stream);

typedef struct dirb200_bn_eval_job {
  int c;
  int64_t gamma_off, beta_off, rm_off, rv_off;
  float* scale;
  float* shift;
} dirb200_bn_eval_job;
int dirb200_bn_eval_coeffs_all(const dirb200_bn_eval_job* jobs_host, int njobs, const float* params,
                               const float* running, float eps, void* stream);

typedef struct dirb200_net dirb200_net;

int dirb200_resnet_create(int n, int h, int w, const int* blocks_per_stage, int num_stages, dirb200_net** out);
void dirb200_resnet_destroy(dirb200_net* net);
int64_t dirb200_resnet_param_count(const dirb200_net* net);
int64_t dirb200_resnet_running_count(const dirb200_net* net);
int64_t dirb200_resnet_feature_dim(const dirb200_net* net);
int64_t dirb200_resnet_device_bytes(const dirb200_net* net);

int dirb200_resnet_forward(dirb200_net* net, const float* x_nchw, const float* params, float* bn_running,
                           int training, float* enc_out, void* stream);

int dirb200_resnet_backward(dirb200_net* net, const float* d_enc, const float* params, float* grads, void* stream);

int dirb200_resnet_num_stages(const dirb200_net* net);
int dirb200_resnet_backward_stage(dirb200_net* net, int stage, const float* d_enc, const float* params, float* grads,
                                  void* stream);
int dirb200_resnet_stage_param_range(const dirb200_net* net, int stage, int64_t* lo, int64_t* hi);

int dirb200_resnet_forward_blocks(dirb200_net* net, const float* x_nchw, const float* params, float* bn_running,
                                  int training, void* const* block_out, void* stream);

int dirb200_resnet_backward_blocks_stage(dirb200_net* net, int stage, const void* d_block, const float* params,
                                         float* grads, void* stream);

int dirb200_resnet_set_profiling(dirb200_net* net, int enabled);
int dirb200_resnet_read_profile(dirb200_net* net, double* ms_by_kind, int64_t* groups_by_kind);

int dirb200_resnet_peek(dirb200_net* net, int block, int which, void** ptr, int64_t* rows, int* channels);

typedef struct dirb200_conv_peek {
  void* w_fprop;
  void* w_dgrad;
  float* partial;
  float* scale;
  float* shift;
  int64_t w_off;
  int cout, cin, kh, kw, stride, pad, stem, splits;
} dirb200_conv_peek;
int dirb200_resnet_peek_conv(dirb200_net* net, int block, int conv, dirb200_conv_peek* out);

int dirb200_resnet_peek_bn_stats(dirb200_net* net, int block, int conv, float** mean, float** invstd);

int dirb200_linear1_fwd(const float* x, const float* w, const float* bias, int64_t n, int d, float* pred,
                        void* stream);
int dirb200_linear1_bwd(const float* grad_pred, const float* x, const float* w, int64_t n, int d, float* dx,
                        float* dw, float* dbias, void* stream);

int dirb200_adam_step(float* params, const float* grads, float* exp_avg, float* exp_avg_sq, int64_t n, float lr,
                      float beta1, float beta2, float eps, float weight_decay, int64_t step, float grad_scale,
                      const float* clip_coef, void* stream);
int dirb200_sgd_step(float* params, const float* grads, float* momentum_buf, int64_t n, float lr, float momentum,
                     float weight_decay, int first_step, float grad_scale, const float* clip_coef, void* stream);

typedef struct dirb200_adam_segment {
  float* param;
  const float* grad;
  float* exp_avg;
  float* exp_avg_sq;
  int64_t numel;
  float bc1;
  float bc2_sqrt;
} dirb200_adam_segment;

int dirb200_adam_step_multi(const dirb200_adam_segment* segs_host, int nseg, float lr, float beta1, float beta2,
                            float eps, float weight_decay, void* stream);
int dirb200_adam_step_multi_clipped(const dirb200_adam_segment* segs_host, int nseg, float lr, float beta1,
                                    float beta2, float eps, float weight_decay, const float* clip_coef, void* stream);

typedef struct dirb200_grad_segment {
  const float* grad;
  int64_t numel;
} dirb200_grad_segment;

size_t dirb200_grad_norm_multi_workspace_bytes(void);
int dirb200_grad_norm_multi(const dirb200_grad_segment* segs_host, int nseg, float max_norm, void* workspace,
                            size_t workspace_bytes, float* out, void* stream);

size_t dirb200_grad_clip_workspace_bytes(void);
int dirb200_grad_clip_coef(const float* grads, int64_t n, float grad_scale, float max_norm, void* workspace,
                           size_t workspace_bytes, float* out, void* stream);

int dirb200_lstm_prep_weights(const float* w_ih_f, const float* w_hh_f, const float* b_ih_f, const float* b_hh_f,
                              const float* w_ih_r, const float* w_hh_r, const float* b_ih_r, const float* b_hh_r,
                              int H, int din, int in_blocks, int Hp, int Dp, void* w_ih, void* w_ih_t, void* w_hh,
                              void* w_hh_t, float* bias, void* stream);
int dirb200_lstm_scatter_grads(const float* dw_ih, const float* dw_hh, const float* db, int H, int din, int in_blocks,
                               int Hp, int Dp, float* gw_ih_f, float* gw_hh_f, float* gb_ih_f, float* gb_hh_f,
                               float* gw_ih_r, float* gw_hh_r, float* gb_ih_r, float* gb_hh_r, void* stream);
int dirb200_lstm_fwd_step(const void* xproj, const void* w_hh, const float* bias, const int* lens, int T, int M,
                          int Hp, int save, int s, void* h, float* c, float* gates, void* y, void* stream);
int dirb200_lstm_layer_fwd(const void* xproj, const void* w_hh, const float* bias, const int* lens, int T, int M,
                           int Hp, int save, void* h, float* c, float* gates, void* y, void* stream);
int dirb200_lstm_bwd_step(const void* w_hh_t, const void* dy, const float* gates, const float* c, const int* lens,
                          int T, int M, int Hp, int s, float* dc, void* dg, void* dg_time, void* stream);
int dirb200_lstm_layer_bwd(const void* w_hh_t, const void* dy, const float* gates, const float* c, const int* lens,
                           int T, int M, int Hp, float* dc, void* dg, void* dg_time, void* stream);
int dirb200_col_sum_bf16(const void* x, int64_t rows, int cols, float* out, void* stream);
int dirb200_embed_gather(const int64_t* ids, const int* lens, const float* emb, const float* dmul, int64_t V, int M,
                         int T, int D, int Dp, void* x, void* stream);
int dirb200_embed_grad(const int64_t* ids, const int* lens, const void* dx, const float* dmul, int64_t V, int M, int T,
                       int D, int Dp, int64_t padding_index, float* dw, void* stream);
int dirb200_pair_maxpool_fwd(const void* y, const int* lens, const float* dmul, int B, int T, int H, int Hp,
                             float* feat, int* arg, void* stream);
int dirb200_pair_maxpool_bwd(const float* gfeat, const float* feat, const int* arg, const float* dmul, int B, int T,
                             int H, int Hp, void* dy, void* stream);

#ifdef __cplusplus
}
#endif
#endif
```

Before: 7680.

## Add optional 256-row implicit-GEMM tiles and tiled transpose for dgrad weight prep

Adds a ROWS template parameter so TMA-fed fprop/dgrad implicit-GEMM kernels can use 256-row M tiles. Each consumer warpgroup issues two m64 wgmma per k step, and setmaxnreg moves registers from producer to consumer warps. The 256-row path is only taken when forced through a new API (g_rows_forced defaults to 0), so by default the kernels still use BM rows. The dgrad weight-transpose prep loop is also rewritten to go through a shared-memory 32x32 tile, which makes its global accesses coalesced; that part runs by default but only costs something at weight-prep time.

```diff
diff --git a/imbalanced-regression_b200/_convlib.py b/imbalanced-regression_b200/_convlib.py
--- a/imbalanced-regression_b200/_convlib.py
+++ b/imbalanced-regression_b200/_convlib.py
@@ -13,6 +13,8 @@
     "dirb200_conv_wgrad_workspace_bytes": (c_size_t, _I9 + [c_int]),
     "dirb200_conv_wgrad": (c_int, [P, P, P, P, c_size_t] + _I9 + [c_int, c_int, P]),
     "dirb200_conv_plan": (c_int, _I9 + [c_int, c_int, P]),
+    "dirb200_conv_tile_rows": (c_int, _I9 + [c_int, c_int, P]),
+    "dirb200_conv_force_tile_rows": (c_int, [c_int]),
     "dirb200_bn_eval_coeffs": (c_int, [c_int, P, P, c_float, P, P, P, P, P]),
     "dirb200_conv_fprop_bn_stats": (c_int, [P, P, P] + _I9 + [c_int, P, P, P]),
     "dirb200_conv_fprop_affine": (c_int, [P, P, P] + _I9 + [P, P, P, c_int, P]),
diff --git a/imbalanced-regression_b200/csrc/conv.cuh b/imbalanced-regression_b200/csrc/conv.cuh
--- a/imbalanced-regression_b200/csrc/conv.cuh
+++ b/imbalanced-regression_b200/csrc/conv.cuh
@@ -48,17 +48,18 @@
   size_t w_off;
   int cout, cin, kh, kw, stem;
   __nv_bfloat16 *wf, *wd;
-  FastDiv fd_cin, fd_cout, fd_taps;
+  FastDiv fd_cin, fd_taps;
 };
 inline PrepDesc make_prep_desc(size_t w_off, int cout, int cin, int kh, int kw, int stem, __nv_bfloat16* wf,
                                __nv_bfloat16* wd) {
-  PrepDesc d{w_off, cout, cin, kh, kw, stem, wf, wd, {}, {}, {}};
+  PrepDesc d{w_off, cout, cin, kh, kw, stem, wf, wd, {}, {}};
   d.fd_cin = make_fastdiv((uint32_t)cin);
-  d.fd_cout = make_fastdiv((uint32_t)cout);
   d.fd_taps = make_fastdiv((uint32_t)(kh * kw));
   return d;
 }
 int conv_plan(const ConvShape& s, bool stem, int op, int* plan);
+int conv_tile_rows(const ConvShape& s, bool stem, int op);
+int conv_force_tile_rows(int rows);
 int prep_weights_all(const float* params, const PrepDesc* descs_dev, int nlayers, cudaStream_t st);
 int prep_weights(const float* w, int cout, int cin, int kh, int kw, bool stem, __nv_bfloat16* wf, __nv_bfloat16* wd,
                  cudaStream_t st);
diff --git a/imbalanced-regression_b200/csrc/conv_api.cu b/imbalanced-regression_b200/csrc/conv_api.cu
--- a/imbalanced-regression_b200/csrc/conv_api.cu
+++ b/imbalanced-regression_b200/csrc/conv_api.cu
@@ -155,11 +155,19 @@
     d.wf[i] = __float2bfloat16_rn(w[((size_t)co * d.cin + c) * taps + tap]);
   }
   if (!d.wd) return;
-  for (uint32_t i = blockIdx.x * blockDim.x + threadIdx.x; i < total; i += stride) {
-    uint32_t t, c, co, tap;
-    d.fd_cout.divmod(i, t, co);
-    d.fd_taps.divmod(t, c, tap);
-    d.wd[i] = __float2bfloat16_rn(w[((size_t)co * d.cin + c) * taps + tap]);
+  __shared__ float tile[32][33];
+  const uint32_t J = (uint32_t)d.cin * taps;
+  const uint32_t tiles_j = (J + 31) / 32, tiles = tiles_j * (((uint32_t)d.cout + 31) / 32);
+  const uint32_t tx = threadIdx.x & 31, ty = threadIdx.x >> 5, rows = blockDim.x >> 5;
+  for (uint32_t t = blockIdx.x; t < tiles; t += gridDim.x) {
+    const uint32_t j0 = (t % tiles_j) * 32, co0 = (t / tiles_j) * 32;
+    __syncthreads();
+    for (uint32_t r = ty; r < 32; r += rows)
+      if (co0 + r < (uint32_t)d.cout && j0 + tx < J) tile[r][tx] = w[(size_t)(co0 + r) * J + j0 + tx];
+    __syncthreads();
+    for (uint32_t r = ty; r < 32; r += rows)
+      if (j0 + r < J && co0 + tx < (uint32_t)d.cout)
+        d.wd[(size_t)(j0 + r) * d.cout + co0 + tx] = __float2bfloat16_rn(tile[tx][r]);
   }
 }
 
@@ -347,6 +355,18 @@
   if (int rc = to_shape(n, h, w, cin, cout, kh, kw, stride, pad, stem, &s)) return rc;
   return conv_plan(s, stem != 0, op, plan7);
 }
+
+int dirb200_conv_tile_rows(int n, int h, int w, int cin, int cout, int kh, int kw, int stride, int pad, int stem, int op,
+                           int* rows_out) {
+  DIRB_CHECK_ARG(rows_out && op >= 0 && op <= 2, "conv_tile_rows: bad arguments");
+  DIRB_CHECK_ARG(!(op == 1 && stem), "conv_tile_rows: the stem has no data gradient");
+  ConvShape s;
+  if (int rc = to_shape(n, h, w, cin, cout, kh, kw, stride, pad, stem, &s)) return rc;
+  *rows_out = conv_tile_rows(s, stem != 0, op);
+  return DIRB200_OK;
+}
+
+int dirb200_conv_force_tile_rows(int rows) { return conv_force_tile_rows(rows); }
 
 int dirb200_prep_weights_all(const float* params, const dirb200_prep_job* jobs_host, int njobs, void* stream) {
   DIRB_CHECK_ARG(params && jobs_host, "prep_weights_all: null pointer");
diff --git a/imbalanced-regression_b200/csrc/conv_igemm.cu b/imbalanced-regression_b200/csrc/conv_igemm.cu
--- a/imbalanced-regression_b200/csrc/conv_igemm.cu
+++ b/imbalanced-regression_b200/csrc/conv_igemm.cu
@@ -46,15 +46,16 @@
   const float* bst_shift;
 };
 
-template <int BN, bool STAGED_EPI>
+template <int BN, bool STAGED_EPI, int ROWS = BM>
 struct Cfg {
-  static constexpr int kABytes = BM * BK * 2;
+  static constexpr int kABytes = ROWS * BK * 2;
   static constexpr int kBBytes = BN * BK * 2;
   static constexpr int kStageBytes = kABytes + kBBytes;
-  static constexpr int kStages = BN == 128 ? (STAGED_EPI ? 5 : 6) : 8;
+  static constexpr int kStages = ROWS == 256 ? (BN == 128 ? 3 : 4) : (BN == 128 ? (STAGED_EPI ? 5 : 6) : 8);
   static constexpr int kBarOffset = kStages * kStageBytes;
   static constexpr int kStageRowBytes = BN * 2 + 16;
-  static constexpr int kEpiWarpBytes = 16 * kStageRowBytes;
+  static constexpr int kEpiRows = 16 * ROWS / 128;
+  static constexpr int kEpiWarpBytes = kEpiRows * kStageRowBytes;
   static constexpr int kEpiOffset = kBarOffset + 256;
   static constexpr int kStatWarpBytes = 2 * BN * 4;
   static constexpr int kStatOffset = kEpiOffset + (STAGED_EPI ? 8 * kEpiWarpBytes : 0);
@@ -114,12 +115,14 @@
   return ok ? P.src + (static_cast<size_t>(rp.nb + hi) * P.ws + wi) * P.cs + coff : P.src;
 }
 
-template <int BN, bool WGRAD, bool STEM, bool ATMA = false, bool AFFINE = false, bool BSTAT = false>
+template <int BN, bool WGRAD, bool STEM, bool ATMA = false, bool AFFINE = false, bool BSTAT = false, int ROWS = BM>
 __global__ void __launch_bounds__(kThreads, 1)
 igemm_kernel(const __grid_constant__ CUtensorMap tmap_b, const __grid_constant__ CUtensorMap tmap_a,
              const IgemmParams P) {
-  using C = Cfg<BN, !WGRAD>;
-  static_assert(BN == 64 || BN == 128, "tile width: one m64n64 / m64n128 wgmma per warpgroup and k step");
+  using C = Cfg<BN, !WGRAD, ROWS>;
+  static_assert(BN == 64 || BN == 128, "tile width: one m64n64 / m64n128 wgmma per m64 row block and k step");
+  static_assert(ROWS == BM || (ROWS == 256 && ATMA && !WGRAD), "256-row tiles: TMA-fed fprop / dgrad only");
+  constexpr int MH = ROWS / 128;
   static_assert(!ATMA || !STEM, "TMA-fed A operand: not for the stem");
   static_assert(!AFFINE || (!WGRAD && !STEM), "folded-BN epilogue: non-stem fprop GEMMs only");
   static_assert(!BSTAT || (ATMA && !WGRAD && !AFFINE), "BN-backward moments in the epilogue: TMA-fed dgrad GEMMs only");
@@ -175,6 +178,7 @@
   __syncthreads();
 
   if (warp < 4) {
+    if constexpr (ROWS == 256) setmaxnreg_dec<40>();
     if constexpr (!ATMA) {
       const int j = lane & 7;
       const int q = lane >> 3;
@@ -332,7 +336,7 @@
         if constexpr (!WGRAD) {
           if (P.a_mode == 2) {
             uint32_t tn, rem, y0, x0;
-            P.fd_hw.divmod(static_cast<uint32_t>(m_tile) * BM, tn, rem);
+            P.fd_hw.divmod(static_cast<uint32_t>(m_tile) * ROWS, tn, rem);
             P.fd_wm.divmod(rem, y0, x0);
             tile_n0 = static_cast<int>(tn);
             tile_w0 = static_cast<int>(x0) * P.i2c_stride + P.i2c_lo;
@@ -349,7 +353,7 @@
             if constexpr (!WGRAD) {
               mbar_arrive_expect_tx(full_bar(s), C::kBBytes + C::kABytes);
               if (P.a_mode == 1)
-                tma_load_2d(a_addr(s), &tmap_a, full_bar(s), kb * BK, m_tile * BM);
+                tma_load_2d(a_addr(s), &tmap_a, full_bar(s), kb * BK, m_tile * ROWS);
               else
                 tma_load_im2col_4d(a_addr(s), &tmap_a, full_bar(s), cb * BK, tile_w0, tile_h0, tile_n0,
                                    P.tap_s[tc], P.tap_r[tc]);
@@ -389,6 +393,7 @@
     return;
   }
 
+  if constexpr (ROWS == 256) setmaxnreg_inc<232>();
   const int g = (warp >> 2) - 1;
   const int wq = warp & 3;
   const int ew = g * 4 + wq;
@@ -401,7 +406,7 @@
   constexpr uint32_t kLbo = WGRAD ? 8192u : 16u;
   constexpr uint32_t kadv = WGRAD ? (2048u >> 4) : (32u >> 4);
   constexpr int kT = WGRAD ? 1 : 0;
-  float acc[BN / 2];
+  float acc[MH][BN / 2];
   uint32_t rs = 0, rph = 0;
   for (int t = tile_first; t < tile_end; t += tile_step) {
     int split, m_tile, n_tile, kb_begin, nk;
@@ -412,16 +417,20 @@
       mbar_wait(full_bar(s), rph);
       if (++rs == nstages) { rs = 0; rph ^= 1u; }
       if constexpr (!ATMA) fence_proxy_async();
-      const uint64_t adesc = make_smem_desc(a_addr(s) + g * 8192, kLbo, 1024u);
+      const uint64_t adesc = make_smem_desc(a_addr(s) + g * MH * 8192, kLbo, 1024u);
       const uint64_t bdesc = make_smem_desc(b_addr(s), kLbo, 1024u);
-      wgmma_fence_operands(acc);
+#pragma unroll
+      for (int h = 0; h < MH; ++h) wgmma_fence_operands(acc[h]);
       wgmma_fence();
 #pragma unroll
       for (int k = 0; k < BK / 16; ++k)
-        wgmma_bf16<BN, kT, kT>(acc, adesc + static_cast<uint64_t>(k * kadv), bdesc + static_cast<uint64_t>(k * kadv),
-                               (it > 0 || k > 0) ? 1u : 0u);
+#pragma unroll
+        for (int h = 0; h < MH; ++h)
+          wgmma_bf16<BN, kT, kT>(acc[h], adesc + static_cast<uint64_t>(k * kadv + h * 512),
+                                 bdesc + static_cast<uint64_t>(k * kadv), (it > 0 || k > 0) ? 1u : 0u);
       wgmma_commit();
-      wgmma_fence_operands(acc);
+#pragma unroll
+      for (int h = 0; h < MH; ++h) wgmma_fence_operands(acc[h]);
       if (it > 0) {
         wgmma_wait<1>();
         if (lane == 0) mbar_arrive(empty_bar(prev));
@@ -429,7 +438,8 @@
       prev = s;
     }
     wgmma_wait<0>();
-    wgmma_fence_operands(acc);
+#pragma unroll
+    for (int h = 0; h < MH; ++h) wgmma_fence_operands(acc[h]);
     if (nk > 0 && lane == 0) mbar_arrive(empty_bar(prev));
     const int n0 = n_tile * BN;
 
@@ -439,30 +449,37 @@
 #pragma unroll
       for (int j = 0; j < BN / 8; ++j) {
         const int col = 8 * j + fc;
-        float v0 = acc[4 * j], v1 = acc[4 * j + 1], v2 = acc[4 * j + 2], v3 = acc[4 * j + 3];
+        float2 a = make_float2(0.f, 0.f), b = a;
         if constexpr (AFFINE) {
-          const float2 a = __ldg(reinterpret_cast<const float2*>(P.epi_scale + n0 + col));
-          const float2 b = __ldg(reinterpret_cast<const float2*>(P.epi_shift + n0 + col));
-          v0 = fmaf(v0, a.x, b.x); v1 = fmaf(v1, a.y, b.y); v2 = fmaf(v2, a.x, b.x); v3 = fmaf(v3, a.y, b.y);
-          if (relu_now) { v0 = fmaxf(v0, 0.f); v1 = fmaxf(v1, 0.f); v2 = fmaxf(v2, 0.f); v3 = fmaxf(v3, 0.f); }
+          a = __ldg(reinterpret_cast<const float2*>(P.epi_scale + n0 + col));
+          b = __ldg(reinterpret_cast<const float2*>(P.epi_shift + n0 + col));
         }
-        __nv_bfloat162 h0 = __floats2bfloat162_rn(v0, v1), h1 = __floats2bfloat162_rn(v2, v3);
-        asm volatile("st.shared.b32 [%0], %1;" ::"r"(stage_base + fr * C::kStageRowBytes + col * 2),
-                     "r"(*reinterpret_cast<uint32_t*>(&h0)) : "memory");
-        asm volatile("st.shared.b32 [%0], %1;" ::"r"(stage_base + (fr + 8) * C::kStageRowBytes + col * 2),
-                     "r"(*reinterpret_cast<uint32_t*>(&h1)) : "memory");
+#pragma unroll
+        for (int mb = 0; mb < MH; ++mb) {
+          float v0 = acc[mb][4 * j], v1 = acc[mb][4 * j + 1], v2 = acc[mb][4 * j + 2], v3 = acc[mb][4 * j + 3];
+          if constexpr (AFFINE) {
+            v0 = fmaf(v0, a.x, b.x); v1 = fmaf(v1, a.y, b.y); v2 = fmaf(v2, a.x, b.x); v3 = fmaf(v3, a.y, b.y);
+            if (relu_now) { v0 = fmaxf(v0, 0.f); v1 = fmaxf(v1, 0.f); v2 = fmaxf(v2, 0.f); v3 = fmaxf(v3, 0.f); }
+          }
+          __nv_bfloat162 h0 = __floats2bfloat162_rn(v0, v1), h1 = __floats2bfloat162_rn(v2, v3);
+          const uint32_t row0 = stage_base + (16 * mb + fr) * C::kStageRowBytes + col * 2;
+          asm volatile("st.shared.b32 [%0], %1;" ::"r"(row0), "r"(*reinterpret_cast<uint32_t*>(&h0)) : "memory");
+          asm volatile("st.shared.b32 [%0], %1;" ::"r"(row0 + 8 * C::kStageRowBytes),
+                       "r"(*reinterpret_cast<uint32_t*>(&h1)) : "memory");
+        }
       }
       __syncwarp();
       constexpr int kLanesPerRow = BN * 2 / 16;
       constexpr int kRowsPerIter = 32 / kLanesPerRow;
-      constexpr int kIters = 16 / kRowsPerIter;
+      constexpr int kIters = C::kEpiRows / kRowsPerIter;
       const int sub = lane / kLanesPerRow, col16 = lane % kLanesPerRow;
-      const long long p0 = static_cast<long long>(m_tile) * BM + g * 64 + wq * 16;
+      const long long p0 = static_cast<long long>(m_tile) * ROWS + g * MH * 64 + wq * 16;
+      auto staged_pixel = [&](int rl) { return p0 + (rl >> 4) * 64 + (rl & 15); };
       __nv_bfloat16* out_cols = reinterpret_cast<__nv_bfloat16*>(P.out) + n0 + col16 * 8;
 #pragma unroll
       for (int i = 0; i < kIters; ++i) {
         const int rl = i * kRowsPerIter + sub;
-        const long long p = p0 + rl;
+        const long long p = staged_pixel(rl);
         int orow = (p < P.pixels && nk > 0) ? static_cast<int>(p) : -1;
         if (orow >= 0 && P.cls_on) {
           const uint32_t pk = pack_pixel(p, P);
@@ -503,13 +520,13 @@
             bsc = __ldg(reinterpret_cast<const float2*>(P.bst_scale + n0 + col));
             bsh = __ldg(reinterpret_cast<const float2*>(P.bst_shift + n0 + col));
           }
-#pragma unroll
-          for (int r = 0; r < 16; ++r) {
+#pragma unroll 16
+          for (int r = 0; r < C::kEpiRows; ++r) {
             uint32_t w;
             asm volatile("ld.shared.b32 %0, [%1];" : "=r"(w) : "r"(stage_base + r * C::kStageRowBytes + col * 2));
             float g0 = __uint_as_float(w << 16), g1 = __uint_as_float(w & 0xffff0000u);
             if constexpr (BSTAT) {
-              const long long p = p0 + r;
+              const long long p = staged_pixel(r);
               const uint32_t yw = p < P.pixels ? __ldg(reinterpret_cast<const unsigned int*>(P.bst_y + p * P.ldc + n0 + col)) : 0u;
               const float y0 = __uint_as_float(yw << 16), y1 = __uint_as_float(yw & 0xffff0000u);
               if (!(fmaf(y0, bsc.x, bsh.x) > 0.f)) g0 = 0.f;
@@ -537,8 +554,8 @@
         const size_t c0 = static_cast<size_t>(8 * j + fc) * ktot;
 #pragma unroll
         for (int e = 0; e < 2; ++e) {
-          if (krow < ktot) out[c0 + e * ktot + krow] = nk > 0 ? acc[4 * j + e] : 0.f;
-          if (krow + 8 < ktot) out[c0 + e * ktot + krow + 8] = nk > 0 ? acc[4 * j + 2 + e] : 0.f;
+          if (krow < ktot) out[c0 + e * ktot + krow] = nk > 0 ? acc[0][4 * j + e] : 0.f;
+          if (krow + 8 < ktot) out[c0 + e * ktot + krow + 8] = nk > 0 ? acc[0][4 * j + 2 + e] : 0.f;
         }
       }
     }
@@ -668,33 +685,38 @@
   return Q;
 }
 
-template <int BN, bool WGRAD, bool STEM, bool ATMA = false, bool AFFINE = false, bool BSTAT = false>
+template <int BN, bool WGRAD, bool STEM, bool ATMA = false, bool AFFINE = false, bool BSTAT = false, int ROWS = BM>
 static int launch_igemm_impl(const CUtensorMap& tm, const CUtensorMap& tma, const IgemmParams& Qin, cudaStream_t st) {
-  using C = Cfg<BN, !WGRAD>;
+  using C = Cfg<BN, !WGRAD, ROWS>;
   const IgemmParams Q = finish_params(Qin);
   static bool configured = false;
   if (!configured) {
-    DIRB_CUDA(cudaFuncSetAttribute(igemm_kernel<BN, WGRAD, STEM, ATMA, AFFINE, BSTAT>,
+    DIRB_CUDA(cudaFuncSetAttribute(igemm_kernel<BN, WGRAD, STEM, ATMA, AFFINE, BSTAT, ROWS>,
                                    cudaFuncAttributeMaxDynamicSharedMemorySize, C::kSmemBytes));
     configured = true;
   }
   int grid = Q.num_tiles < num_sms() ? Q.num_tiles : num_sms();
   if (!WGRAD && grid < Q.n_tiles) grid = Q.n_tiles;
   t_last_layout = StatLayout{grid, Q.n_tiles, BN, 1};
-  igemm_kernel<BN, WGRAD, STEM, ATMA, AFFINE, BSTAT><<<grid, kThreads, C::kSmemBytes, st>>>(tm, tma, Q);
+  igemm_kernel<BN, WGRAD, STEM, ATMA, AFFINE, BSTAT, ROWS><<<grid, kThreads, C::kSmemBytes, st>>>(tm, tma, Q);
   DIRB_LAUNCHED();
   return DIRB200_OK;
 }
 
 template <int BN, bool WGRAD, bool STEM>
 static int launch_igemm(const CUtensorMap& tm, const IgemmParams& P, int m_tiles, int splits, cudaStream_t st,
-                        const CUtensorMap* tma = nullptr) {
+                        const CUtensorMap* tma = nullptr, int rows = BM) {
   IgemmParams Q = P;
   Q.m_tiles = m_tiles;
   Q.num_tiles = m_tiles * P.n_tiles * splits;
   if constexpr (!STEM) {
     if (tma) {
       if constexpr (!WGRAD) {
+        if (rows == 256) {
+          if (Q.epi_scale != nullptr) return launch_igemm_impl<BN, false, false, true, true, false, 256>(tm, *tma, Q, st);
+          if (Q.bst_y != nullptr) return launch_igemm_impl<BN, false, false, true, false, true, 256>(tm, *tma, Q, st);
+          return launch_igemm_impl<BN, false, false, true, false, false, 256>(tm, *tma, Q, st);
+        }
         if (Q.epi_scale != nullptr) return launch_igemm_impl<BN, false, false, true, true>(tm, *tma, Q, st);
         if (Q.bst_y != nullptr) return launch_igemm_impl<BN, false, false, true, false, true>(tm, *tma, Q, st);
       }
@@ -745,6 +767,23 @@
     return !(e != nullptr && e[0] == '0');
   }();
   return on && atma_enabled();
+}
+
+static int g_rows_forced = 0;
+
+int conv_tile_rows(const ConvShape& s, bool stem, int op) {
+  if (stem || op == 2 || g_rows_forced == 0) return BM;
+  const bool tma_fed = op == 0 ? (is_plain_gemm(s, stem) || im2col_enabled())
+                               : (s.stride == 1 ? (is_plain_gemm(s, false) || (im2col_enabled() && s.kh == s.kw))
+                                                : im2col_enabled());
+  return tma_fed ? g_rows_forced : BM;
+}
+
+int conv_force_tile_rows(int rows) {
+  DIRB_CHECK_ARG(rows == 0 || rows == 128 || rows == 256, "conv_force_tile_rows: rows must be 0, 128 or 256 (got %d)",
+                 rows);
+  g_rows_forced = rows;
+  return DIRB200_OK;
 }
 
 static int conv_fprop_impl(const __nv_bfloat16* x, const __nv_bfloat16* w, __nv_bfloat16* y, const ConvShape& s, bool stem,
@@ -781,26 +820,27 @@
   if (epi) {
     P.epi_scale = epi->scale; P.epi_shift = epi->shift; P.epi_res = epi->residual; P.epi_relu = epi->relu ? 1 : 0;
   }
-  const int m_tiles = static_cast<int>((P.pixels + BM - 1) / BM);
+  const int rows = conv_tile_rows(s, stem, 0);
+  const int m_tiles = static_cast<int>((P.pixels + rows - 1) / rows);
   const int bn = pick_bn(s.cout);
   P.n_tiles = s.cout / bn;
   CUtensorMap tm, ta;
   bool tma_fed = false;
   if (is_plain_gemm(s, stem)) {
-    if (int rc = make_tmap_bf16_2d(&ta, x, s.cin, static_cast<uint64_t>(P.pixels), static_cast<uint64_t>(s.cin) * 2, BM))
+    if (int rc = make_tmap_bf16_2d(&ta, x, s.cin, static_cast<uint64_t>(P.pixels), static_cast<uint64_t>(s.cin) * 2, rows))
       return rc;
     P.a_mode = 1;
     tma_fed = true;
   } else if (!stem && im2col_enabled()) {
     if (int rc = make_tmap_im2col_bf16(&ta, x, s.cin, s.w, s.h, s.n, -s.pad, -s.pad, s.pad - (s.kw - 1),
-                                       s.pad - (s.kh - 1), s.stride, BM))
+                                       s.pad - (s.kh - 1), s.stride, rows))
       return rc;
     P.a_mode = 2; P.i2c_stride = s.stride; P.i2c_lo = -s.pad;
     tma_fed = true;
   }
   if (int rc = make_tmap_bf16_2d(&tm, w, ktot, s.cout, static_cast<uint64_t>(ktot) * 2, bn)) return rc;
   if (stem) return DISPATCH_BN(bn, false, true, tm, P, m_tiles, 1, st);
-  if (tma_fed) return DISPATCH_BN(bn, false, false, tm, P, m_tiles, 1, st, &ta);
+  if (tma_fed) return DISPATCH_BN(bn, false, false, tm, P, m_tiles, 1, st, &ta, rows);
   return DISPATCH_BN(bn, false, false, tm, P, m_tiles, 1, st);
 }
 
@@ -826,6 +866,7 @@
     P.bst_y = bnm->y; P.bst_scale = bnm->scale; P.bst_shift = bnm->shift; P.stat_out = bnm->partial;
   }
   const int bn = pick_bn(s.cin);
+  const int rows = conv_tile_rows(s, false, 1);
   CUtensorMap tm;
   if (int rc = make_tmap_bf16_2d(&tm, wt, ktot, s.cin, static_cast<uint64_t>(ktot) * 2, bn)) return rc;
   if (s.stride == 1) {
@@ -833,23 +874,23 @@
     P.ntaps_c = s.kh * s.kw;
     for (int i = 0; i < kMaxTaps; ++i) P.tap_list[i] = i;
     P.num_kblocks = ktot / 64;
-    const int m_tiles = static_cast<int>((P.pixels + BM - 1) / BM);
+    const int m_tiles = static_cast<int>((P.pixels + rows - 1) / rows);
     P.n_tiles = s.cin / bn;
     CUtensorMap ta;
     bool tma_fed = false;
     if (is_plain_gemm(s, false)) {
-      if (int rc = make_tmap_bf16_2d(&ta, dy, s.cout, static_cast<uint64_t>(P.pixels), static_cast<uint64_t>(s.cout) * 2, BM))
+      if (int rc = make_tmap_bf16_2d(&ta, dy, s.cout, static_cast<uint64_t>(P.pixels), static_cast<uint64_t>(s.cout) * 2, rows))
         return rc;
       P.a_mode = 1;
       tma_fed = true;
     } else if (im2col_enabled() && s.kh == s.kw) {
       const int lo = s.pad - (s.kh - 1);
-      if (int rc = make_tmap_im2col_bf16(&ta, dy, s.cout, s.wo, s.ho, s.n, lo, lo, lo + s.w - s.wo, lo + s.h - s.ho, 1, BM))
+      if (int rc = make_tmap_im2col_bf16(&ta, dy, s.cout, s.wo, s.ho, s.n, lo, lo, lo + s.w - s.wo, lo + s.h - s.ho, 1, rows))
         return rc;
       P.a_mode = 2; P.i2c_stride = 1; P.i2c_lo = lo;
       tma_fed = true;
     }
-    const int rc = tma_fed ? DISPATCH_BN(bn, false, false, tm, P, m_tiles, 1, st, &ta)
+    const int rc = tma_fed ? DISPATCH_BN(bn, false, false, tm, P, m_tiles, 1, st, &ta, rows)
                            : DISPATCH_BN(bn, false, false, tm, P, m_tiles, 1, st);
     if (bnm && bnm->layout) *bnm->layout = t_last_layout;
     return rc;
@@ -877,7 +918,7 @@
     if (Q.ntaps_c == 0 || Q.hm <= 0 || Q.wm <= 0) continue;
     Q.pixels = static_cast<long long>(s.n) * Q.hm * Q.wm;
     Q.num_kblocks = Q.ntaps_c * Q.cpb;
-    const int m_tiles = static_cast<int>((Q.pixels + BM - 1) / BM);
+    const int m_tiles = static_cast<int>((Q.pixels + rows - 1) / rows);
     Q.n_tiles = s.cin / bn;
     if (im2col_enabled()) {
       int lo = 1 << 20;
@@ -888,10 +929,10 @@
         lo = oq < lo ? oq : lo;
       }
       CUtensorMap ta;
-      if (int rc = make_tmap_im2col_bf16(&ta, dy, s.cout, s.wo, s.ho, s.n, lo, lo, lo + Q.wm - s.wo, lo + Q.hm - s.ho, 1, BM))
+      if (int rc = make_tmap_im2col_bf16(&ta, dy, s.cout, s.wo, s.ho, s.n, lo, lo, lo + Q.wm - s.wo, lo + Q.hm - s.ho, 1, rows))
         return rc;
       Q.a_mode = 2; Q.i2c_stride = 1; Q.i2c_lo = lo;
-      if (int rc = DISPATCH_BN(bn, false, false, tm, Q, m_tiles, 1, st, &ta)) return rc;
+      if (int rc = DISPATCH_BN(bn, false, false, tm, Q, m_tiles, 1, st, &ta, rows)) return rc;
       continue;
     }
     if (int rc = DISPATCH_BN(bn, false, false, tm, Q, m_tiles, 1, st)) return rc;
diff --git a/imbalanced-regression_b200/csrc/tc.cuh b/imbalanced-regression_b200/csrc/tc.cuh
--- a/imbalanced-regression_b200/csrc/tc.cuh
+++ b/imbalanced-regression_b200/csrc/tc.cuh
@@ -81,6 +81,17 @@
       : "memory");
 }
 
+template <uint32_t N>
+__device__ __forceinline__ void setmaxnreg_dec() {
+  static_assert(N >= 24 && N <= 256 && N % 8 == 0, "setmaxnreg: 24 .. 256 in steps of 8");
+  asm volatile("setmaxnreg.dec.sync.aligned.u32 %0;" ::"n"(N));
+}
+template <uint32_t N>
+__device__ __forceinline__ void setmaxnreg_inc() {
+  static_assert(N >= 24 && N <= 256 && N % 8 == 0, "setmaxnreg: 24 .. 256 in steps of 8");
+  asm volatile("setmaxnreg.inc.sync.aligned.u32 %0;" ::"n"(N));
+}
+
 __device__ __forceinline__ void wgmma_fence() { asm volatile("wgmma.fence.sync.aligned;" ::: "memory"); }
 __device__ __forceinline__ void wgmma_commit() { asm volatile("wgmma.commit_group.sync.aligned;" ::: "memory"); }
 template <int N>
diff --git a/include/dirb200.h b/include/dirb200.h
--- a/include/dirb200.h
+++ b/include/dirb200.h
@@ -156,6 +156,9 @@
 
 int dirb200_conv_plan(int n, int h, int w, int cin, int cout, int kh, int kw, int stride, int pad, int stem, int op,
                       int* plan7);
+int dirb200_conv_tile_rows(int n, int h, int w, int cin, int cout, int kh, int kw, int stride, int pad, int stem, int op,
+                           int* rows_out);
+int dirb200_conv_force_tile_rows(int rows);
 size_t dirb200_conv_wgrad_workspace_bytes(int n, int h, int w, int cin, int cout, int kh, int kw,
                                           int stride, int pad, int stem);
 
```

Result: no change. 7707, median of 6 (+0.4%).
